# balaji1312/cassnat_asr_public

Measured on AMD Instinct MI355X. Metric: utterances_per_sec, higher is better.
Workload: dtype bf16; 1 GPU; BASELINE configs[1]: CASS-NAT 12L-enc / 1+3+2 dec blocks, d_model 256, 4 heads, d_ff 2048, V 5000, greedy NAST; 32 utterances x 1000 frames x 80 fbank per GPU per step; batch_per_gpu=32, frames=1000, feat_dim=80, global_batch=32, parallelism=utterance-sharded x1, decode_pipelines_per_gpu=2, batches_per_engine_pass=10, utterances_per_engine_pass=320, row_predictions=208, row_predictions_missed=0

## Files before the change

cassnat_asr_public_amd/abi.py:

```python
import ctypes as C
import os
import re

HEADER_PATH = os.path.join(os.path.dirname(os.path.dirname(os.path.abspath(__file__))), "include", "cassnat_hip.h")
SCALARS = {"int": C.c_int, "int32_t": C.c_int32, "int64_t": C.c_int64, "uint64_t": C.c_uint64, "float": C.c_float, "double": C.c_double}
_BASE = re.compile(r"(?:const\s+)?(\w+)\s*")
_DECL = re.compile(r"((?:\*\s*)*)(\w*)\s*(?:\[(\d+)\])?")


class AbiError(ValueError):
    pass


class Abi:
    def __init__(self):
        self.functions, self.structs, self.constants, self.opaque = {}, {}, {}, set()

    def ctype(self, base, stars, where):
        if not stars and base in SCALARS:
            return SCALARS[base]
        if stars == 1 and base == "char":
            return C.c_char_p
        if stars == 1 and base in self.structs:
            return C.POINTER(self.structs[base])
        if stars and (base in SCALARS or base in self.structs or base in self.opaque or base in ("void", "char", "uint8_t")):
            return C.c_void_p
        raise AbiError(f"{where}: unknown type {base + '*' * stars!r}")

    def declarators(self, text, where):
        text = " ".join(text.split())
        m = _BASE.match(text)
        out = []
        for part in text[m.end():].split(",") if m else ():
            d = _DECL.fullmatch(part.strip())
            if not d:
                raise AbiError(f"{where}: cannot read {text!r}")
            if m.group(1) == "void" and not d.group(1) and not d.group(2):
                out.append(("", None))
                continue
            t = self.ctype(m.group(1), d.group(1).count("*"), f"{where}: {text!r}")
            out.append((d.group(2), t * int(d.group(3)) if d.group(3) else t))
        if not out:
            raise AbiError(f"{where}: cannot read {text!r}")
        return out


def parse(text, base=None):
    abi = Abi()
    if base is not None:
        abi.structs.update(base.structs)
        abi.opaque.update(base.opaque)
    text = re.sub(r"/\*.*?\*/|//[^\n]*", " ", text, flags=re.S)
    for name, value in re.findall(r"^[ \t]*#[ \t]*define[ \t]+(CN_\w+)[ \t]+(-?\w+)[ \t]*$", text, re.M):
        abi.constants[name] = int(value, 0)
    text = re.sub(r'^[ \t]*#[^\n]*|extern\s+"C"\s*\{', " ", text, flags=re.M)

    def enum(m):
        for item in filter(None, (s.strip() for s in m.group(1).split(","))):
            name, eq, value = (s.strip() for s in item.partition("="))
            if not eq or not re.fullmatch(r"\w+", name):
                raise AbiError(f"enum: cannot read {item!r}")
            abi.constants[name] = int(value, 0)
        return " "

    def struct(m):
        fields = []
        for line in filter(None, (s.strip() for s in m.group(2).split(";"))):
            got = abi.declarators(line, f"struct {m.group(1)}")
            if any(not name or t is None for name, t in got):
                raise AbiError(f"struct {m.group(1)}: cannot read {line!r}")
            fields += got
        cls = "".join(p.title() for p in m.group(1).split("_"))
        abi.structs[m.group(1)] = type(cls, (C.Structure,), {"_fields_": fields, "__doc__": f"{m.group(1)} of include/cassnat_hip.h"})
        return " "

    text = re.sub(r"\benum\s*\{(.*?)\}\s*;", enum, text, flags=re.S)
    abi.opaque.update(re.findall(r"\btypedef\s+struct\s+(\w+)\s+\1\s*;", text))
    text = re.sub(r"\btypedef\s+struct\s+(\w+)\s+\1\s*;", " ", text)
    text = re.sub(r"\btypedef\s+struct\s+(\w+)\s*\{(.*?)\}\s*\1\s*;", struct, text, flags=re.S)
    for stmt in filter(None, (s.strip() for s in text.split(";"))):
        m = re.fullmatch(r"(.*?)\b(cn_\w+)\s*\((.*)\)", stmt, re.S)
        if not m:
            if stmt == "}":
                continue
            raise AbiError(f"cannot split the declaration {' '.join(stmt.split())!r}")
        name, params = m.group(2), m.group(3).strip()
        ret = abi.declarators(m.group(1), f"{name}: return type")
        args = [] if params == "void" else [d for p in params.split(",") for d in abi.declarators(p, name)]
        if len(ret) != 1 or ret[0][0] or any(not n or t is None for n, t in args):
            raise AbiError(f"cannot split the declaration of {name}: {' '.join(stmt.split())!r}")
        abi.functions[name] = (ret[0][1], [t for _, t in args])
    return abi


with open(HEADER_PATH) as _f:
    HEADER = parse(_f.read())
FUNCTIONS, STRUCTS, CONSTANTS = HEADER.functions, HEADER.structs, HEADER.constants
EXTRA_HEADER_PATH = os.path.join(os.path.dirname(HEADER_PATH), "cassnat_hip_ctc_ngram.h")
with open(EXTRA_HEADER_PATH) as _f:
    EXTRA_FUNCTIONS = parse(_f.read(), base=HEADER).functions


def bind(L):
    for name, (restype, argtypes) in list(FUNCTIONS.items()) + list(EXTRA_FUNCTIONS.items()):
        fn = getattr(L, name)
        fn.restype, fn.argtypes = restype, argtypes
    return L
```

cassnat_asr_public_amd/build.py:

```python
import os
import shutil
import subprocess
import sys
from concurrent.futures import ThreadPoolExecutor

CSRC = os.path.join(os.path.dirname(os.path.abspath(__file__)), "csrc")
LIB = os.path.join(os.path.dirname(os.path.abspath(__file__)), "libcassnat_hip.so")
LIB_F16 = os.path.join(os.path.dirname(os.path.abspath(__file__)), "libcassnat_hip_f16.so")
SOURCES = ["gemm.hip", "fbank.hip", "resample.hip", "flac.hip", "conv2.hip", "conv1.hip", "rowops.hip", "attention.hip", "ctc_align.hip", "ctc_beam.hip", "fused.hip", "fused_x3.hip", "genmax.hip", "proj_x3.hip", "conformer.hip", "chain.hip", "ast.hip", "natlm.hip", "ctc_lm.hip", "ngram.hip", "ctc_ngram.hip", "model.hip", "handle.hip", "weights.hip", "workspace.hip", "sublayers.hip", "decode_ar.hip", "ops.hip"]
FLAGS = ["--offload-arch=gfx950", "-O3", "-std=c++17", "-fPIC", "-Wall", "-Wno-unused-function"]
FILE_FLAGS = {"conv1.hip": ["-mllvm", "-amdgpu-mfma-vgpr-form=1"]}


def _hipcc():
    return shutil.which("hipcc") or "/opt/rocm/bin/hipcc"


def _stale(target, deps):
    if not os.path.exists(target):
        return True
    t = os.path.getmtime(target)
    return any(os.path.getmtime(d) > t for d in deps)


def build(force=False, verbose=False, extra_flags=(), lib=LIB, objdir=None):
    headers = [os.path.join(CSRC, h) for h in os.listdir(CSRC) if h.endswith(".h")]
    headers += [os.path.join(os.path.dirname(CSRC), "..", "include", h) for h in ("cassnat_hip.h", "cassnat_hip_ctc_ngram.h")]
    objdir = objdir or os.path.join(CSRC, "build")
    os.makedirs(objdir, exist_ok=True)

    def compile_one(src):
        obj = os.path.join(objdir, src.replace(".hip", ".o"))
        path = os.path.join(CSRC, src)
        if force or _stale(obj, [path] + headers):
            cmd = [_hipcc()] + FLAGS + FILE_FLAGS.get(src, []) + list(extra_flags) + ["-c", path, "-o", obj]
            if verbose:
                print(" ".join(cmd), file=sys.stderr)
            r = subprocess.run(cmd, capture_output=True, text=True)
            if r.returncode != 0:
                raise RuntimeError(f"hipcc failed on {src}:\n{r.stderr}")
        return obj

    with ThreadPoolExecutor(max_workers=min(6, len(SOURCES))) as ex:
        objs = list(ex.map(compile_one, SOURCES))
    if force or _stale(lib, objs):
        cmd = [_hipcc(), "--offload-arch=gfx950", "-shared", "-fPIC", "-o", lib] + objs
        r = subprocess.run(cmd, capture_output=True, text=True)
        if r.returncode != 0:
            raise RuntimeError(f"link failed:\n{r.stderr}")
    return lib


def build_f16(force=False, verbose=False):
    return build(force=force, verbose=verbose, extra_flags=["-DCN_OP16_F16"], lib=LIB_F16, objdir=os.path.join(CSRC, "build_f16"))


def build_all(force=False, verbose=False):
    return build(force=force, verbose=verbose), build_f16(force=force, verbose=verbose)


def experiments_lib(extra_flags=(), tag="exp"):
    root = os.path.join(os.path.dirname(os.path.dirname(os.path.abspath(__file__))), "ab")
    os.makedirs(root, exist_ok=True)
    return build(extra_flags=["-DCASSNAT_EXPERIMENTS"] + list(extra_flags), lib=os.path.join(root, "libcassnat_hip_%s.so" % tag),
                 objdir=os.path.join(root, "obj_" + tag))


if __name__ == "__main__":
    if "--experiments" in sys.argv:
        print(experiments_lib())
        sys.exit(0)
    for path in build_all(force="--force" in sys.argv, verbose=True):
        print(path)
```

cassnat_asr_public_amd/csrc/attention.hip:

```cpp
#include <cstdlib>

#include <cstdio>
#include <cstdlib>

#include "kernels.h"

struct AttnParams {
    const unsigned char* Q;
    const unsigned char* K;
    const unsigned char* V;
    void* O;
    long long ldq_b, ldk_b, ldv_b;
    int ldo;
    int H, Lq, Lk;
    const unsigned char* keymask;
    int kv_mod;
    int stamps;
    const int* kv_index;
    const int* klen;
    int o_blk;
    int q_blk, kv_blk;
    int q_col, k_col, v_col, q_n, kv_n;
    const int* kcap;
    int kcap_stride;
    const int* iv;
    int iv_stride;
    int causal;
    float scale;
    const float* rel_pos;
    const float* rel_u;
    const float* rel_v;
    int rel_R, ld_pos;
    const int* row_off;
    int kv_packed;
};

template <typename T> struct AttnCfg;
template <> struct AttnCfg<bf16> {
    static constexpr int KROW = 128;
    static constexpr int VROW = 192;
    static constexpr int CPR = 8;
    __device__ static int swz(int row) { return (row >> 1) & 7; }
};
template <> struct AttnCfg<float> {
    static constexpr int KROW = 256;
    static constexpr int VROW = 256;
    static constexpr int CPR = 16;
    __device__ static int swz(int row) { return row & 15; }
};

template <> struct AttnCfg<split_t> {
    static constexpr int KROW = 256;
    static constexpr int VROW = 192;
    static constexpr int CPR = 16;
    __device__ static int swz(int row) { return row & 15; }
};

__device__ long long attn_stamps[8];
#define AT_STAMP(i) if (p.stamps && blockIdx.x == 0 && blockIdx.y == gridDim.y - 1 && blockIdx.z == gridDim.z - 1 && threadIdx.x == 0) attn_stamps[i] = (long long)__builtin_amdgcn_s_memtime();

template <typename T, int NW, bool RES, bool REL = false, bool PK = false>
__global__ __launch_bounds__(64 * NW, (RES && NW == 8) ? 4 : ((__is_same(T, split_t) && NW == 4 && !REL) ? 2 : 1)) void attention_kernel(AttnParams p) {
    typedef AttnCfg<T> Cfg;
    typedef typename Frag<T>::type frag_t;
    constexpr bool SPLIT = __is_same(T, split_t);
    static_assert(!SPLIT || !RES, "split-bf16 attention: the staged forms only");
    constexpr int KROW = Cfg::KROW, CPR = Cfg::CPR;
    constexpr int VROW = RES ? 128 : Cfg::VROW;
    constexpr int KT_BYTES = 64 * KROW, VT_BYTES = (SPLIT ? 2 : 1) * 64 * VROW, NRES = RES ? 4 : 1;
    constexpr int NF = SPLIT ? 4 : KROW / 32;
    constexpr int NT = 64 * NW;
    constexpr int ST_IT = 64 * CPR / NT;

    __shared__ __attribute__((aligned(16))) unsigned char Ks_all[NRES * KT_BYTES];
    __shared__ __attribute__((aligned(16))) unsigned char Vs_all[NRES * VT_BYTES];
    __shared__ __attribute__((aligned(16))) unsigned int Ms_all[NRES * 16];
    __shared__ unsigned int Mplain[NRES];

    const int tid = threadIdx.x, lane = tid & 63, wave = tid >> 6;
    const int half = lane >> 5, l31 = lane & 31;
    const int b = blockIdx.z, h = blockIdx.y;
    AT_STAMP(0)
    const long long q0 = PK ? (long long)p.row_off[b] : (long long)b * p.Lq;
    const int Lq = PK ? p.row_off[b + 1] - p.row_off[b] : p.Lq;
    if constexpr (PK) {
        if ((int)blockIdx.x * (32 * NW) >= Lq) return;
    }
    const int q_row = blockIdx.x * (32 * NW) + wave * 32 + l31;
    const bool wave_active = (blockIdx.x * (32 * NW) + wave * 32) < Lq;
    const int qc = q_row < Lq ? q_row : Lq - 1;

    frag_t qf[NF];
    {
        const unsigned char* qp = p.Q + (q0 + qc) * p.ldq_b + (long long)h * KROW;
        if constexpr (SPLIT) {
#pragma unroll
            for (int s = 0; s < NF; ++s) {
                const unsigned char* c = qp + (s >> 1) * 128 + (2 * (s & 1) + half) * 16;
                qf[s].hi = as_frag<bf16>(ld16(c));
                qf[s].lo = as_frag<bf16>(ld16(c + 64));
            }
        } else if constexpr (PK) {
            const long long qm = q0 + qc;
#pragma unroll
            for (int s = 0; s < NF; ++s) {
                const unsigned char* src = qp + (2 * s + half) * 16;
                src = p.q_blk ? p.Q + cn_blk16_off(qm, p.q_col + h * 64 + (2 * s + half) * 8, p.q_n) : src;
                qf[s] = as_frag<T>(ld16(src));
            }
        } else if (p.q_blk) {
            const long long qm = q0 + qc;
#pragma unroll
            for (int s = 0; s < NF; ++s) qf[s] = as_frag<T>(ld16(p.Q + cn_blk16_off(qm, p.q_col + h * 64 + (2 * s + half) * 8, p.q_n)));
        } else {
#pragma unroll
            for (int s = 0; s < NF; ++s) qf[s] = as_frag<T>(ld16(qp + (2 * s + half) * 16));
        }
    }
    constexpr int REL_N = REL ? 64 : 1;
    __shared__ float rel_tab[REL ? 64 * 64 : 1];
    __shared__ float rel_bias[REL ? NW : 1][32][REL_N];
    if constexpr (REL) {
        constexpr int E = SPLIT ? 8 : Frag<T>::ELEMS;
        const int nr = 2 * p.rel_R + 1;
        for (int i = tid; i < nr * 64; i += NT) rel_tab[i] = p.rel_pos[(long long)(i >> 6) * p.ld_pos + h * 64 + (i & 63)];
        __syncthreads();
        auto dim_of = [&](int s, int j) -> int {
            if constexpr (SPLIT) return 32 * (s >> 1) + 16 * (s & 1) + 8 * half + j;
            else return (2 * s + half) * E + j;
        };
        float qv[NF][E];
#pragma unroll
        for (int s = 0; s < NF; ++s)
#pragma unroll
            for (int j = 0; j < E; ++j) {
                const int dim = dim_of(s, j);
                if constexpr (SPLIT) {
                    const float q = (float)qf[s].hi[j] + (float)qf[s].lo[j];
                    qv[s][j] = q + p.rel_v[h * 64 + dim];
                    const float qu = q + p.rel_u[h * 64 + dim];
                    const bf16 hi = (bf16)qu;
                    qf[s].hi[j] = hi;
                    qf[s].lo[j] = (bf16)(qu - (float)hi);
                } else {
                    const float q = to_f32(qf[s][j]);
                    qv[s][j] = q + p.rel_v[h * 64 + dim];
                    qf[s][j] = from_f32<T>(q + p.rel_u[h * 64 + dim]);
                }
            }
        for (int r = 0; r < nr; ++r) {
            float acc = 0.f;
#pragma unroll
            for (int s = 0; s < NF; ++s)
#pragma unroll
                for (int j = 0; j < E; ++j) acc = fmaf(qv[s][j], rel_tab[r * 64 + dim_of(s, j)], acc);
            acc += __shfl_xor(acc, 32);
            if (half == 0) rel_bias[wave][l31][r] = acc;
        }
        __syncthreads();
    }
    int iv_s1 = 0, iv_e1 = 0, iv_s2 = 0, iv_e2 = 0;
    if (p.iv) {
        const int4 r = *reinterpret_cast<const int4*>(p.iv + ((long long)b * p.iv_stride + qc) * 4);
        iv_s1 = r.x;
        iv_e1 = r.y;
        iv_s2 = r.z;
        iv_e2 = r.w;
    }
    const int klen = p.klen ? p.klen[b] : p.Lk;
    unsigned char* Ks = Ks_all;
    unsigned char* Vs = Vs_all;
    unsigned int* Ms = Ms_all;

    uint4 k_reg[ST_IT], v_reg[ST_IT];
    const int bk = p.kv_index ? p.kv_index[b] : (p.kv_mod > 0 ? b % p.kv_mod : b);
    const bool kpk = PK && p.kv_packed;
    const long long k0 = kpk ? (long long)p.row_off[bk] : (long long)bk * p.Lk;
    const int krows = kpk ? p.row_off[bk + 1] - p.row_off[bk] : p.Lk;
    int kcap = p.kcap ? p.kcap[(long long)bk * p.kcap_stride] : p.Lk;
    if (krows < kcap) kcap = krows;
    const int kvalid = kcap < p.Lk ? kcap : p.Lk;
    const int nkt = kvalid > 0 ? (kvalid + 63) / 64 : 1;
    const unsigned char* kbase = p.K + k0 * p.ldk_b + (long long)h * KROW;
    const unsigned char* vbase = p.V + k0 * p.ldv_b + (long long)h * KROW;
    auto load_tile = [&](int kt) {
#pragma unroll
        for (int i = 0; i < ST_IT; ++i) {
            const int cidx = tid + NT * i;
            const int row = cidx / CPR, ch = cidx % CPR;
            const int key = kt * 64 + row;
            if (key < krows) {
                if (p.kv_blk) {
                    const long long km = k0 + key;
                    k_reg[i] = ld16(p.K + cn_blk16_off(km, p.k_col + h * 64 + ch * 8, p.kv_n));
                    v_reg[i] = ld16(p.V + cn_blk16_off(km, p.v_col + h * 64 + ch * 8, p.kv_n));
                } else {
                    k_reg[i] = ld16(kbase + (long long)key * p.ldk_b + ch * 16);
                    v_reg[i] = ld16(vbase + (long long)key * p.ldv_b + ch * 16);
                }
            } else {
                k_reg[i] = make_uint4(0, 0, 0, 0);
                v_reg[i] = make_uint4(0, 0, 0, 0);
            }
        }
    };
    auto store_tile = [&](int kt) {
#pragma unroll
        for (int i = 0; i < ST_IT; ++i) {
            const int cidx = tid + NT * i;
            const int row = cidx / CPR, ch = cidx % CPR;
            st16(Ks + row * KROW + ((ch ^ Cfg::swz(row)) << 4), k_reg[i]);
            if constexpr (SPLIT)
                st16(Vs + ((ch >> 2) & 1) * 64 * VROW + row * VROW + ((((ch >> 3) << 2) | (ch & 3)) << 4), v_reg[i]);
            else
                st16(Vs + row * VROW + (ch << 4), v_reg[i]);
        }
        if (tid < 64) {
            const int key = kt * 64 + tid;
            unsigned char code = 2;
            if (key < kcap) {
                bool ok = key < klen;
                if (p.keymask) ok = ok && p.keymask[(long long)bk * p.Lk + key] != 0;
                code = ok ? 1 : 0;
            }
            reinterpret_cast<unsigned char*>(Ms)[tid] = code;
            const unsigned long long bad0 = __ballot(code == 0), bad2 = __ballot(code == 2);
            if (tid == 0) Mplain[0] = 1u | (bad2 != 0ull ? 2u : 0u) | (bad0 != 0ull ? 4u : 0u);
        }
    };

    f32x16 o_acc[2];
#pragma unroll
    for (int d = 0; d < 2; ++d)
#pragma unroll
        for (int r = 0; r < 16; ++r) o_acc[d][r] = 0.f;
    float m_run = CN_NEG_FILL, l_run = 0.f;

    if constexpr (RES) {
        const int wave_u = __builtin_amdgcn_readfirstlane(wave);
        const int r8 = lane >> 3, cp = lane & 7;
        for (int piece = wave_u; piece < nkt * 16; piece += NW) {
            const int kt2 = piece >> 4, is_v = (piece >> 3) & 1, j = piece & 7;
            const int row = 8 * j + r8;
            int key = kt2 * 64 + row;
            if (key >= krows) key = krows - 1;
            const int chunk = is_v ? (cp ^ (((row >> 1) & 1) << 2)) : (cp ^ Cfg::swz(row));
            const unsigned char* src;
            if (p.kv_blk)
                src = (is_v ? p.V : p.K) + cn_blk16_off(k0 + key, (is_v ? p.v_col : p.k_col) + h * 64 + chunk * 8, p.kv_n);
            else
                src = is_v ? vbase + (long long)key * p.ldv_b + (chunk << 4) : kbase + (long long)key * p.ldk_b + (chunk << 4);
            unsigned char* dst = (is_v ? Vs_all + kt2 * VT_BYTES : Ks_all + kt2 * KT_BYTES) + j * 1024;
            __builtin_amdgcn_global_load_lds((const __attribute__((address_space(1))) void*)src,
                                             (__attribute__((address_space(3))) void*)dst, 16, 0, 0);
        }
        AT_STAMP(1)
        if (tid < NRES) Mplain[tid] = 1;
        __syncthreads();
        for (int i = tid; i < nkt * 64; i += NT) {
            unsigned char code = 2;
            if (i < kcap) {
                bool ok = i < klen;
                if (p.keymask) ok = ok && p.keymask[(long long)bk * p.Lk + i] != 0;
                code = ok ? 1 : 0;
            }
            reinterpret_cast<unsigned char*>(Ms_all)[i] = code;
            if (code != 1) atomicOr(&Mplain[i >> 6], code == 2 ? 2u : 4u);
        }
        asm volatile("s_waitcnt vmcnt(0)" ::: "memory");
        __syncthreads();
        AT_STAMP(2)
    } else {
        load_tile(0);
    }
    for (int kt = 0; kt < nkt; ++kt) {
        if constexpr (RES) {
            Ks = Ks_all + kt * KT_BYTES;
            Vs = Vs_all + kt * VT_BYTES;
            Ms = Ms_all + kt * 16;
        } else {
            __syncthreads();
            store_tile(kt);
            __syncthreads();
            if (kt + 1 < nkt) load_tile(kt + 1);
        }
        if (!wave_active) continue;

        const unsigned tile_class = Mplain[RES ? kt : 0];
        const bool simple = !REL && !p.iv && !p.causal && (tile_class & 4u) == 0;
#pragma unroll
        for (int sub = 0; sub < 2; ++sub) {
            if (simple && kt * 64 + sub * 32 >= kcap) continue;
            f32x16 sc;
#pragma unroll
            for (int r = 0; r < 16; ++r) sc[r] = 0.f;
            {
                const int row = sub * 32 + l31;
#pragma unroll
                for (int s = 0; s < NF; ++s) {
                    if constexpr (SPLIT) {
                        const int chunk = (s >> 1) * 8 + 2 * (s & 1) + half;
                        split_frag kf;
                        kf.hi = as_frag<bf16>(ld16(Ks + row * KROW + ((chunk ^ Cfg::swz(row)) << 4)));
                        kf.lo = as_frag<bf16>(ld16(Ks + row * KROW + (((chunk + 4) ^ Cfg::swz(row)) << 4)));
                        sc = mfma_frag(kf, qf[s], sc);
                    } else {
                        const int chunk = 2 * s + half;
                        const frag_t kf = as_frag<T>(ld16(Ks + row * KROW + ((chunk ^ Cfg::swz(row)) << 4)));
                        sc = mfma_frag(kf, qf[s], sc);
                    }
                }
            }
            float psum = 0.f, alpha;
            const bool plain = simple && kt * 64 + sub * 32 + 32 <= kcap;
            if (simple) {
                float tmax;
                if (plain) {
                    tmax = sc[0];
#pragma unroll
                    for (int r = 1; r < 16; ++r) tmax = fmaxf(tmax, sc[r]);
                } else {
                    const int k0 = kt * 64 + sub * 32 + 4 * half;
                    tmax = -INFINITY;
#pragma unroll
                    for (int r = 0; r < 16; ++r) {
                        sc[r] = k0 + 8 * (r >> 2) + (r & 3) < kcap ? sc[r] : -INFINITY;
                        tmax = fmaxf(tmax, sc[r]);
                    }
                }
                tmax = xhalf_max(tmax) * p.scale;
                const float m_new = fmaxf(m_run, tmax);
                alpha = __expf(m_run - m_new);
                m_run = m_new;
                const float c2 = p.scale * 1.44269504088896340736f, mb = m_new * 1.44269504088896340736f;
#pragma unroll
                for (int r = 0; r < 16; ++r) {
                    const float pv = __builtin_amdgcn_exp2f(fmaf(sc[r], c2, -mb));
                    sc[r] = pv;
                    psum += pv;
// ... 147 lines not shown
            }
        }
        return;
    }
    if (q_row < Lq) {
        T* orow = reinterpret_cast<T*>(p.O) + (q0 + q_row) * p.ldo + h * 64;
#pragma unroll
        for (int d = 0; d < 2; ++d) {
#pragma unroll
            for (int g = 0; g < 4; ++g) {
                const int dk0 = 32 * d + 8 * g + 4 * half;
                if constexpr (SPLIT) {
                    float o[4];
#pragma unroll
                    for (int e = 0; e < 4; ++e) o[e] = o_acc[d][4 * g + e] * inv;
                    bf16x4 hi, lo;
                    cn_split4(o, hi, lo);
                    unsigned char* ob = reinterpret_cast<unsigned char*>(orow) + cn_split_off((size_t)dk0);
                    *reinterpret_cast<bf16x4*>(ob) = hi;
                    *reinterpret_cast<bf16x4*>(ob + 64) = lo;
                } else if constexpr (sizeof(T) == 2) {
                    bf16x4 o;
#pragma unroll
                    for (int e = 0; e < 4; ++e) o[e] = (bf16)(o_acc[d][4 * g + e] * inv);
                    *reinterpret_cast<bf16x4*>(orow + dk0) = o;
                } else {
                    f32x4 o;
#pragma unroll
                    for (int e = 0; e < 4; ++e) o[e] = o_acc[d][4 * g + e] * inv;
                    *reinterpret_cast<f32x4*>(orow + dk0) = o;
                }
            }
        }
    }
    AT_STAMP(4)
}

int attention_print_stamps() {
    long long h[8];
    CN_HIP_CHECK(hipMemcpyFromSymbol(h, HIP_SYMBOL(attn_stamps), sizeof(h)));
    static const char* names[] = {"", "Q fragments + K/V requests", "K/V landed + mask codes", "key-tile loop", "normalise + store"};
    for (int i = 1; i < 5; ++i) fprintf(stderr, "[attention stamps] %-28s %8lld ticks\n", names[i], h[i] - h[i - 1]);
    fprintf(stderr, "[attention stamps] total %lld ticks (s_memtime)\n", h[4] - h[0]);
    return 0;
}

template <typename T> static int run_attention(const AttnArgs& a, hipStream_t s) {
    constexpr bool PKT = sizeof(T) == 2 && !__is_same(T, split_t);
    AttnParams p;
    p.Q = (const unsigned char*)a.Q;
    p.K = (const unsigned char*)a.K;
    p.V = (const unsigned char*)a.V;
    p.O = a.O;
    p.ldq_b = (long long)a.ldq * sizeof(T);
    p.ldk_b = (long long)a.ldk * sizeof(T);
    p.ldv_b = (long long)a.ldv * sizeof(T);
    p.ldo = a.ldo;
    p.H = a.H;
    p.Lq = a.Lq;
    p.Lk = a.Lk;
    p.keymask = a.keymask;
    p.kv_mod = a.kv_mod;
    static const int stamps = cn_exp_env("CASSNAT_ATTN_STAMPS") ? 1 : 0;
    p.stamps = stamps;
    p.kv_index = a.kv_index;
    p.klen = a.klen;
    p.kcap = a.kcap;
    p.kcap_stride = a.kcap_stride;
    p.o_blk = a.o_blocked;
    p.q_blk = a.q_blocked;
    p.kv_blk = a.kv_blocked;
    p.q_col = a.q_col;
    p.k_col = a.k_col;
    p.v_col = a.v_col;
    p.q_n = a.q_n;
    p.kv_n = a.kv_n;
    if ((a.q_blocked || a.kv_blocked || a.o_blocked) && (sizeof(T) != 2 || __is_same(T, split_t) || a.rel_pos || (a.q_blocked && a.q_n % 32) ||
                                          (a.kv_blocked && a.kv_n % 32) || (a.o_blocked && a.ldo % 32))) {
        cn_set_error("attention: blocked operands exist for the bf16 kernels without relative positions; column counts % 32 == 0");
        return -1;
    }
    p.row_off = a.row_off;
    p.kv_packed = a.kv_packed;
    if ((a.row_off && (a.rel_pos || sizeof(T) != 2 || __is_same(T, split_t))) ||
        (a.kv_packed && (!a.row_off || a.kv_mod > 0 || a.kv_index || a.keymask || a.Lq != a.Lk))) {
        cn_set_error("attention: packed rows exist for the 16-bit kernels without relative positions; packed keys are the entry's own "
                     "rows (self attention without a key mask, kv_mod or kv_index)");
        return -1;
    }
    p.iv = a.intervals;
    p.iv_stride = a.iv_stride;
    p.causal = a.causal;
    p.scale = a.scale;
    p.rel_pos = a.rel_pos;
    p.rel_u = a.rel_u;
    p.rel_v = a.rel_v;
    p.rel_R = a.rel_R;
    p.ld_pos = a.ld_pos;
    {
        if (a.rel_pos) {
            if (a.rel_R < 0 || a.rel_R > 31 || !a.rel_u || !a.rel_v || a.Lq != a.Lk) {
                cn_set_error("attention: relative positions need self attention and max_relative_len <= 31");
                return -1;
            }
            hipLaunchKernelGGL((attention_kernel<T, 2, false, true>), dim3(cn_ceil_div(a.Lq, 64), a.H, a.B), dim3(128), 0, s, p);
            CN_HIP_CHECK(hipGetLastError());
            return 0;
        }
    }
    const long long big_grid = (long long)cn_ceil_div(a.Lq, 128) * a.H * a.B;
    if constexpr (sizeof(T) == 2) {
        static const int no_res = cn_exp_env("CASSNAT_ATTN_NO_RES") ? 1 : 0;
        if (a.Lk <= 256 && !no_res) {
            static const int nw = cn_exp_env("CASSNAT_ATTN_NW") ? atoi(cn_exp_env("CASSNAT_ATTN_NW")) : 0;
            const int use = nw ? nw : (a.Lq > 128 ? 8 : (a.Lq > 64 ? 4 : 2));
            if (a.row_off) {
                if (use >= 8)
                    hipLaunchKernelGGL((attention_kernel<T, 8, true, false, PKT>), dim3(cn_ceil_div(a.Lq, 256), a.H, a.B), dim3(512), 0, s, p);
                else if (use >= 4)
                    hipLaunchKernelGGL((attention_kernel<T, 4, true, false, PKT>), dim3(cn_ceil_div(a.Lq, 128), a.H, a.B), dim3(256), 0, s, p);
                else
                    hipLaunchKernelGGL((attention_kernel<T, 2, true, false, PKT>), dim3(cn_ceil_div(a.Lq, 64), a.H, a.B), dim3(128), 0, s, p);
            } else if (use >= 8)
                hipLaunchKernelGGL((attention_kernel<T, 8, true>), dim3(cn_ceil_div(a.Lq, 256), a.H, a.B), dim3(512), 0, s, p);
            else if (use >= 4)
                hipLaunchKernelGGL((attention_kernel<T, 4, true>), dim3(cn_ceil_div(a.Lq, 128), a.H, a.B), dim3(256), 0, s, p);
            else
                hipLaunchKernelGGL((attention_kernel<T, 2, true>), dim3(cn_ceil_div(a.Lq, 64), a.H, a.B), dim3(128), 0, s, p);
            CN_HIP_CHECK(hipGetLastError());
            return 0;
        }
    }
    if (a.row_off) {
        if (big_grid >= 1024)
            hipLaunchKernelGGL((attention_kernel<T, 4, false, false, PKT>), dim3(cn_ceil_div(a.Lq, 128), a.H, a.B), dim3(256), 0, s, p);
        else
            hipLaunchKernelGGL((attention_kernel<T, 2, false, false, PKT>), dim3(cn_ceil_div(a.Lq, 64), a.H, a.B), dim3(128), 0, s, p);
    } else if (big_grid >= 1024)
        hipLaunchKernelGGL((attention_kernel<T, 4, false>), dim3(cn_ceil_div(a.Lq, 128), a.H, a.B), dim3(256), 0, s, p);
    else
        hipLaunchKernelGGL((attention_kernel<T, 2, false>), dim3(cn_ceil_div(a.Lq, 64), a.H, a.B), dim3(128), 0, s, p);
    CN_HIP_CHECK(hipGetLastError());
    return 0;
}

int launch_attention(int prec, const AttnArgs& a, hipStream_t s) {
    if (a.B <= 0 || a.Lq <= 0 || a.Lk <= 0 || a.H <= 0) return 0;
    const size_t es = cn_elem_size(prec);
    if ((a.ldq * es) % 16 || (a.ldk * es) % 16 || (a.ldv * es) % 16 || (a.ldo * es) % 16) {
        cn_set_error("attention: row strides must keep rows 16-byte aligned");
        return -1;
    }
    if (prec == CN_PREC_X3) {
        if (a.ldq % 32 || a.ldk % 32 || a.ldv % 32 || a.ldo % 32) {
            cn_set_error("attention: split-bf16 rows need strides that are multiples of 32 elements");
            return -1;
        }
    }
    const long long w = 64LL * a.H;
    if ((!a.q_blocked && a.ldq < w) || (!a.kv_blocked && (a.ldk < w || a.ldv < w)) || a.ldo < w) {
        cn_set_error("attention: row strides ldq / ldk / ldv / ldo must be >= 64 * H");
        return -1;
    }
    if (a.rel_pos && a.ld_pos < w) {
        cn_set_error("attention: the relative-position table needs ld_pos >= 64 * H");
        return -1;
    }
    auto bad_window = [w](int col, int n) { return col < 0 || col % 8 || col + w > n; };
    if ((a.q_blocked && bad_window(a.q_col, a.q_n)) ||
        (a.kv_blocked && (bad_window(a.k_col, a.kv_n) || bad_window(a.v_col, a.kv_n)))) {
        cn_set_error("attention: a blocked operand's columns col .. col + 64 * H - 1 must lie inside its q_n / kv_n columns "
                     "(col >= 0, col % 8 == 0)");
        return -1;
    }
    if (prec == CN_PREC_X3) return run_attention<split_t>(a, s);
    return prec == CN_PREC_F32 ? run_attention<float>(a, s) : run_attention<bf16>(a, s);
}
```

cassnat_asr_public_amd/csrc/chain.hip:

```cpp
#include <cstdio>
#include <cstdlib>
#include <algorithm>
#include <cmath>
#include <cstring>
#include <vector>

#include "kernels.h"

constexpr int CH_D = 256;
constexpr int CH_UNIT_BYTES = 16384;
constexpr int CH_RING = 8;
constexpr int CH_TAB_FLOATS = 5120;
constexpr int CH_TAB_BYTES = CH_TAB_FLOATS * 4;
constexpr int CH_LDS = CH_TAB_BYTES + CH_RING * CH_UNIT_BYTES;
static_assert(CH_LDS <= 160 * 1024, "LDS budget");
constexpr int CT_BO = 0, CT_LN1A = 256, CT_LN1B = 512, CT_B2 = 768, CT_NLNA = 1024, CT_NLNB = 1280, CT_BT = 1536,
              CT_B1 = 3072;
constexpr int CH_MAX_TAIL = 48, CH_MAX_FFN_TILES = 64;

__device__ long long ch_stamps[16];

typedef unsigned u32x4 __attribute__((ext_vector_type(4)));
typedef int v4i __attribute__((ext_vector_type(4)));
typedef int v8i __attribute__((ext_vector_type(8)));

struct ChainParams {
    float* x;
    const bf16* ctx;
    int ldctx;
    const uint4* wstream;
    const float* tab;
    bf16* out;
    int ldo;
    bf16* ln_out;
    int ld_ln;
    int M, ffn_tiles, tail_tiles, has_next;
    float eps;
    int stamps;
    int stamp_block;
    int x_in_blk, x_out_blk, store_x;
    int out_blk;
    int ctx_blk;
    const int* f8_q;
    const int* m_dev;
};

#define CH_STR2(x) #x
#define CH_STR(x) CH_STR2(x)
#define CH_DMA(src, dst)                                                                              \
    __builtin_amdgcn_global_load_lds((const __attribute__((address_space(1))) void*)(src),          \
                                     (__attribute__((address_space(3))) void*)(dst), 16, 0, 0)
#define CH_READ8(F, addr, OFFK)                                                                       \
    asm volatile("ds_read_b128 %0, %8 offset:" CH_STR(((OFFK) + 0) * 1024) "\n\t"                     \
                 "ds_read_b128 %1, %8 offset:" CH_STR(((OFFK) + 1) * 1024) "\n\t"                     \
                 "ds_read_b128 %2, %8 offset:" CH_STR(((OFFK) + 2) * 1024) "\n\t"                     \
                 "ds_read_b128 %3, %8 offset:" CH_STR(((OFFK) + 3) * 1024) "\n\t"                     \
                 "ds_read_b128 %4, %8 offset:" CH_STR(((OFFK) + 4) * 1024) "\n\t"                     \
                 "ds_read_b128 %5, %8 offset:" CH_STR(((OFFK) + 5) * 1024) "\n\t"                     \
                 "ds_read_b128 %6, %8 offset:" CH_STR(((OFFK) + 6) * 1024) "\n\t"                     \
                 "ds_read_b128 %7, %8 offset:" CH_STR(((OFFK) + 7) * 1024)                            \
                 : "=&v"(F[0]), "=&v"(F[1]), "=&v"(F[2]), "=&v"(F[3]), "=&v"(F[4]), "=&v"(F[5]),      \
                   "=&v"(F[6]), "=&v"(F[7])                                                           \
                 : "v"(addr)                                                                          \
                 : "memory")
#define CH_WAIT8(F)                                                                                   \
    asm volatile("s_waitcnt lgkmcnt(0)"                                                               \
                 : "+v"(F[0]), "+v"(F[1]), "+v"(F[2]), "+v"(F[3]), "+v"(F[4]), "+v"(F[5]), "+v"(F[6]), "+v"(F[7]) \
                 :: "memory")
__device__ __forceinline__ void ch_tab4_nowait(unsigned addr, f32x4& a, f32x4& b, f32x4& c, f32x4& d) {
    asm volatile("ds_read_b128 %0, %4\n\t"
                 "ds_read_b128 %1, %4 offset:32\n\t"
                 "ds_read_b128 %2, %4 offset:64\n\t"
                 "ds_read_b128 %3, %4 offset:96"
                 : "=&v"(a), "=&v"(b), "=&v"(c), "=&v"(d)
                 : "v"(addr)
                 : "memory");
}
template <typename D>
__device__ __forceinline__ void ch_tab4_nowait_after(unsigned addr, const D& dep, f32x4& a, f32x4& b, f32x4& c, f32x4& d) {
    asm volatile("ds_read_b128 %0, %4\n\t"
                 "ds_read_b128 %1, %4 offset:32\n\t"
                 "ds_read_b128 %2, %4 offset:64\n\t"
                 "ds_read_b128 %3, %4 offset:96"
                 : "=&v"(a), "=&v"(b), "=&v"(c), "=&v"(d)
                 : "v"(addr), "v"(dep)
                 : "memory");
}
template <typename D>
__device__ __forceinline__ void ch_tab4(unsigned addr, const D& dep, f32x4& a, f32x4& b, f32x4& c, f32x4& d) {
    asm volatile("ds_read_b128 %0, %4\n\t"
                 "ds_read_b128 %1, %4 offset:32\n\t"
                 "ds_read_b128 %2, %4 offset:64\n\t"
                 "ds_read_b128 %3, %4 offset:96\n\t"
                 "s_waitcnt lgkmcnt(0)"
                 : "=&v"(a), "=&v"(b), "=&v"(c), "=&v"(d)
                 : "v"(addr), "v"(dep)
                 : "memory");
}

#define CH_SB0_ __builtin_amdgcn_sched_barrier(0)
#define CH_LGKM_WAIT4(N, a, b, c, d) asm volatile("s_waitcnt lgkmcnt(" #N ")" : "+v"(a), "+v"(b), "+v"(c), "+v"(d) :: "memory")

template <bool ADD>
__device__ __forceinline__ void ch_layernorm_pack(f32x16 (&acc)[8], unsigned tab_lane, int off_a, int off_b, int off_add,
                                                  float eps, bf16x8 (&bop)[16]) {
    float s = 0.f;
#pragma unroll
    for (int nt = 0; nt < 8; ++nt)
#pragma unroll
        for (int r = 0; r < 16; ++r) s += acc[nt][r];
    s += __shfl_xor(s, 32);
    const float mean = s / (float)CH_D;
    float ss = 0.f;
#pragma unroll
    for (int nt = 0; nt < 8; ++nt)
#pragma unroll
        for (int r = 0; r < 16; ++r) ss = fmaf(acc[nt][r] - mean, acc[nt][r] - mean, ss);
    ss += __shfl_xor(ss, 32);
    const float inv = 1.0f / (sqrtf(ss / (float)(CH_D - 1)) + eps);
    f32x4 ga[2][4], be[2][4], ad[2][4];
    CH_SB0_;
    ch_tab4_nowait_after(tab_lane + off_a * 4, inv, ga[0][0], ga[0][1], ga[0][2], ga[0][3]);
    ch_tab4_nowait(tab_lane + off_b * 4, be[0][0], be[0][1], be[0][2], be[0][3]);
    if constexpr (ADD) ch_tab4_nowait(tab_lane + off_add * 4, ad[0][0], ad[0][1], ad[0][2], ad[0][3]);
#pragma unroll
    for (int nt = 0; nt < 8; ++nt) {
        const int c = nt & 1, n = c ^ 1;
// ... 621 lines not shown
        CH_ACT_GAP(HAS_OLD, XO, 5)                                                                             \
        CH_M1(XN, Fa[6], bop[6]);                                                                              \
        CH_ACT_GAP(HAS_OLD, XO, 6)                                                                             \
        CH_M1(XN, Fa[7], bop[7]);                                                                              \
        CH_ACT_GAP(HAS_OLD, XO, 7)                                                                             \
        CH_BLK1("+", "v", "%[c]", XN, Fb, bop, 8, Fa, RA_B, RK_B, CH_PRE_B_##k(M0OFF), CH_DMA0(SOFF), CH_DMA1, CH_DMA2, \
                CH_DMA3, SB, CH_NODRAIN);                                                                      \
        ch_tab4_nowait(tabb(TNEXT), b1v[0], b1v[1], b1v[2], b1v[3]);
#define CH_W2N(k, RA_A, RK_A, RA_B, RK_B, M0OFF, SOFF, SB, PREA, POST)                                        \
        CH_BLK2(acc, Fa, pb[0], Fb, RA_A, RK_A, PREA, "", "", "", "", SB, CH_NODRAIN);                         \
        CH_BLK2(acc, Fb, pb[1], Fa, RA_B, RK_B, CH_PRE_B_##k(M0OFF), CH_DMA0(SOFF), CH_DMA1, CH_DMA2, CH_DMA3, SB, POST);
#define CH_FFN_GROUP(FIRST, LAST)                                                                              \
        {                                                                                                      \
            const uint4* sb_cur = group_base(gpos);                                                            \
            const uint4* sb_next = group_base(gpos + 1);                                                       \
            const int t0 = 4 * g;                                                                              \
            if constexpr (FIRST) {                                                                             \
                CH_W1N(0, ra0, 8, ra0, 16, 0x1C000, 0x1C000, sb_cur, xh0, xh1, false, 1)                       \
                 \
                 \
                 \
                asm volatile("s_nop 13\n\ts_nop 13\n\ts_waitcnt lgkmcnt(0)" : "+v"(xh0), "+v"(b1v[0]), "+v"(b1v[1]), "+v"(b1v[2]), "+v"(b1v[3]), "+v"(Fa[0]), \
                             "+v"(Fa[1]), "+v"(Fa[2]), "+v"(Fa[3]), "+v"(Fa[4]), "+v"(Fa[5]), "+v"(Fa[6]), "+v"(Fa[7]) :: "memory"); \
            } else {                                                                                           \
                CH_W2N(0, ra0, 8, ra0, 16, 0x1C000, 0x1C000, sb_cur, CH_PRE_A4, CH_NODRAIN)                    \
            }                                                                                                  \
            CH_W1N(1, ra0, 24, ra0, 32, 0x0, 0x0, sb_next, xh1, xh0, true, t0 + 2)                             \
            CH_W2N(2, ra0, 40, ra0, 48, 0x4000, 0x4000, sb_next, CH_PRE_A4, CH_NODRAIN)                        \
            CH_W1N(3, ra0, 56, ra1, 0, 0x8000, 0x8000, sb_next, xh0, xh1, true, t0 + 3)                        \
            CH_W2N(4, ra1, 8, ra1, 16, 0xC000, 0xC000, sb_next, CH_PRE_A4, CH_NODRAIN)                         \
            CH_W1N(5, ra1, 24, ra1, 32, 0x10000, 0x10000, sb_next, xh1, xh0, true, t0 + 4)                     \
            CH_W2N(6, ra1, 40, ra1, 48, 0x14000, 0x14000, sb_next, CH_PRE_A4, CH_NODRAIN)                      \
            if constexpr (!(LAST)) {                                                                           \
                CH_W1N(7, ra1, 56, ra0, 0, 0x18000, 0x18000, sb_next, xh0, xh1, true, t0 + 5)                  \
            } else {                                                                                           \
                 \
                 \
                 \
                asm volatile("" : "+v"(xh1));                                                                  \
                CH_SB0;                                                                                        \
                _Pragma("unroll") for (int i = 0; i < 8; ++i) CH_ACT_PIECE(xh1, i)                             \
                CH_SB0;                                                                                        \
                CH_W2N(7, ra1, 56, ra0, 0, 0x18000, 0x18000, sb_next, CH_PRE_A, CH_DRAIN "s_waitcnt lgkmcnt(0)\n\t") \
            }                                                                                                  \
            ++g;                                                                                               \
            ++gpos;                                                                                            \
        }
        int g = 0;
        if (G_FFN == 1) {
            CH_FFN_GROUP(true, true)
        } else {
            CH_FFN_GROUP(true, false)
            while (g < G_FFN - 1) CH_FFN_GROUP(false, false)
            CH_FFN_GROUP(false, true)
        }
#undef CH_FFN_GROUP
#undef CH_W1N
#undef CH_W2N
#undef CH_ACT_GAP
#undef CH_ACT_PIECE
        CH_LAND_FRAGMENTS("");
        asm volatile("s_waitcnt lgkmcnt(0)" : "+v"(b1v[0]), "+v"(b1v[1]), "+v"(b1v[2]), "+v"(b1v[3]) :: "memory");
    }
    CH_STAMP(5)

    if (p.store_x && (p.x_out_blk ? rb < nrb : live)) {
        float* xp = p.x_out_blk ? p.x + (long long)rb * 8192 + 4 * lane : p.x + (long long)m * CH_D + 4 * half;
        const int step = p.x_out_blk ? 256 : 8;
#pragma unroll
        for (int nt = 0; nt < 8; ++nt)
#pragma unroll
            for (int g = 0; g < 4; ++g) {
                f32x4 o;
#pragma unroll
                for (int e = 0; e < 4; ++e) o[e] = acc[nt][4 * g + e];
                *reinterpret_cast<f32x4*>(xp + step * (4 * nt + g)) = o;
            }
    }
    CH_STAMP(6)
    if (p.has_next) {
        ch_layernorm_pack<false>(acc, tab_lane, CT_NLNA, CT_NLNB, 0, p.eps, bop);
        CH_STAMP(7)
        if (p.ln_out) {
            if (live) {
                bf16* op = p.ln_out + (long long)m * p.ld_ln + 4 * half;
#pragma unroll
                for (int k = 0; k < 16; ++k)
#pragma unroll
                    for (int q = 0; q < 2; ++q) {
                        bf16x4 o;
#pragma unroll
                        for (int e = 0; e < 4; ++e) o[e] = bop[k][4 * q + e];
                        *reinterpret_cast<bf16x4*>(op + 16 * k + 8 * q) = o;
                    }
            }
        }
        if (G_TAIL > 0) {
            f32x16 q0, q1;
            f32x4 btv[4];
            bf16x4 o_[4];
            u32x4 w_[2];
            const int NTT = 8 * G_TAIL;
            auto tabt = [&](int tt) -> unsigned { return tab_lane + (unsigned)((CT_BT + 32 * (tt < NTT ? tt : NTT - 1)) * 4); };
            bf16* op16 = p.out + (long long)m * p.ldo + 8 * half;
            unsigned char* ob16 = reinterpret_cast<unsigned char*>(p.out) + (long long)rb * (p.ldo >> 5) * 2048 + lane * 16;
            unsigned char* st_base = p.out_blk ? ob16 : reinterpret_cast<unsigned char*>(op16);
            const int st_tile = p.out_blk ? 2048 : 64, st_half = p.out_blk ? 1024 : 32;
            const bool st_on = (p.out_blk ? rb < nrb : live) && p.stamps != 2;
            ch_tab4_nowait(tabt(0), btv[0], btv[1], btv[2], btv[3]);
            CH_READ8(Fa, ra0, 0);
            asm volatile("s_waitcnt lgkmcnt(0)" : "+v"(btv[0]), "+v"(btv[1]), "+v"(btv[2]), "+v"(btv[3]), "+v"(Fa[0]), "+v"(Fa[1]),
                         "+v"(Fa[2]), "+v"(Fa[3]), "+v"(Fa[4]), "+v"(Fa[5]), "+v"(Fa[6]), "+v"(Fa[7]) :: "memory");
#define CH_TAIL_STORE(v, ptr) *(ptr) = (v)
#define CH_EPI_CVT(QO, g0)                                                                                     \
            {                                                                                                  \
                _Pragma("unroll") for (int g_ = (g0); g_ < (g0) + 2; ++g_)                                     \
                    _Pragma("unroll") for (int e = 0; e < 4; ++e) o_[g_][e] = (bf16)QO[4 * g_ + e];             \
                asm volatile("" : "+v"(o_[g0]), "+v"(o_[(g0) + 1]));                                            \
            }
#define CH_EPI_OUT(TT, gp)                                                                                     \
            {                                                                                                  \
                const uint2 lo_ = __builtin_bit_cast(uint2, o_[2 * (gp)]), hi_ = __builtin_bit_cast(uint2, o_[2 * (gp) + 1]); \
                const auto s0_ = __builtin_amdgcn_permlane32_swap(lo_.x, hi_.x, false, false);                 \
                const auto s1_ = __builtin_amdgcn_permlane32_swap(lo_.y, hi_.y, false, false);                 \
                w_[gp] = u32x4{s0_[0], s1_[0], s0_[1], s1_[1]};                                                \
                if (st_on) CH_TAIL_STORE(w_[gp], reinterpret_cast<u32x4*>(st_base + (long long)(TT) * st_tile + (gp) * st_half)); \
                else asm volatile("" :: "v"(w_[gp]));                                                          \
            }
#define CH_EPI_GAP(HAS_OLD, CODE)                                                                              \
            CH_SB0;                                                                                            \
            if constexpr (HAS_OLD) CODE                                                                        \
            CH_SB0;
#define CH_S5N(k, RA_A, RK_A, RA_B, RK_B, M0OFF, SOFF, SB, QN, QO, HAS_OLD)                                    \
            QN = __builtin_shufflevector(__builtin_shufflevector(btv[0], btv[1], 0, 1, 2, 3, 4, 5, 6, 7),      \
                                         __builtin_shufflevector(btv[2], btv[3], 0, 1, 2, 3, 4, 5, 6, 7),      \
                                         0, 1, 2, 3, 4, 5, 6, 7, 8, 9, 10, 11, 12, 13, 14, 15);   \
            CH_M1R(CH_PRE_A, QN, Fa[0], bop[0], Fb[0], Fb[1], RA_A, (RK_A) + 0);                               \
            CH_SB0;                                                                                            \
            ch_tab4_nowait(tabt(8 * g + (k) + 1), btv[0], btv[1], btv[2], btv[3]);   \
            CH_SB0;                                                                                            \
            CH_M1R("", QN, Fa[1], bop[1], Fb[2], Fb[3], RA_A, (RK_A) + 2);                                     \
            CH_SB0;                                                                                            \
            CH_M1R("", QN, Fa[2], bop[2], Fb[4], Fb[5], RA_A, (RK_A) + 4);                                     \
            CH_EPI_GAP(HAS_OLD, CH_EPI_CVT(QO, 0))                                                             \
            CH_M1R("", QN, Fa[3], bop[3], Fb[6], Fb[7], RA_A, (RK_A) + 6);                                     \
            CH_EPI_GAP(HAS_OLD, CH_EPI_CVT(QO, 2))                                                             \
            CH_M1(QN, Fa[4], bop[4]);                                                                          \
            CH_EPI_GAP(HAS_OLD, CH_EPI_OUT(8 * g + (k) - 1, 0))                                                \
            CH_M1(QN, Fa[5], bop[5]);                                                                          \
            CH_EPI_GAP(HAS_OLD, CH_EPI_OUT(8 * g + (k) - 1, 1))                                                \
            CH_M1(QN, Fa[6], bop[6]);                                                                          \
            CH_SB0;                                                                                            \
            CH_M1(QN, Fa[7], bop[7]);                                                                          \
            CH_SB0;                                                                                            \
            CH_BLK1("+", "v", "%[c]", QN, Fb, bop, 8, Fa, RA_B, RK_B, CH_PRE_B_##k(M0OFF), CH_DMA0(SOFF), CH_DMA1, CH_DMA2, \
                    CH_DMA3, SB, CH_NODRAIN);
#define CH_TAIL_GROUP(FIRST, LAST)                                                                             \
            {                                                                                                  \
                const uint4* sb_cur = group_base(gpos);                                                        \
                const uint4* sb_next = group_base(gpos + 1);                                                   \
                CH_S5N(0, ra0, 8, ra0, 16, 0x1C000, 0x1C000, sb_cur, q0, q1, !(FIRST))                         \
                CH_S5N(1, ra0, 24, ra0, 32, 0x0, 0x0, sb_next, q1, q0, true)                                   \
                CH_S5N(2, ra0, 40, ra0, 48, 0x4000, 0x4000, sb_next, q0, q1, true)                             \
                CH_S5N(3, ra0, 56, ra1, 0, 0x8000, 0x8000, sb_next, q1, q0, true)                              \
                CH_S5N(4, ra1, 8, ra1, 16, 0xC000, 0xC000, sb_next, q0, q1, true)                              \
                CH_S5N(5, ra1, 24, ra1, 32, 0x10000, 0x10000, sb_next, q1, q0, true)                           \
// ... 2 lines not shown
                if constexpr (LAST) {                                                                          \
                       \
                    CH_LAND_FRAGMENTS("");                                                                     \
                    asm volatile(CH_DRAIN : "+v"(q1));                                                         \
                    CH_SB0;                                                                                    \
                    CH_EPI_CVT(q1, 0) CH_EPI_CVT(q1, 2) CH_EPI_OUT(8 * g + 7, 0) CH_EPI_OUT(8 * g + 7, 1)      \
                    CH_SB0;                                                                                    \
                }                                                                                              \
                ++g;                                                                                           \
                ++gpos;                                                                                        \
            }
            int g = 0;
            if (G_TAIL == 1) {
                CH_TAIL_GROUP(true, true)
            } else {
                CH_TAIL_GROUP(true, false)
                while (g < G_TAIL - 1) CH_TAIL_GROUP(false, false)
                CH_TAIL_GROUP(false, true)
            }
#undef CH_TAIL_GROUP
#undef CH_S5N
#undef CH_EPI_GAP
#undef CH_EPI_OUT
#undef CH_EPI_CVT
            CH_LAND_FRAGMENTS("");
            asm volatile("s_waitcnt lgkmcnt(0)" : "+v"(btv[0]), "+v"(btv[1]), "+v"(btv[2]), "+v"(btv[3]) :: "memory");
        }
    }
    CH_STAMP(8)
    asm volatile("s_waitcnt vmcnt(0) lgkmcnt(0)" ::: "memory");
    CH_STAMP(9)
    if (p.stamps && (int)blockIdx.x == p.stamp_block && tid == 0) ch_stamps[11] = (long long)__builtin_amdgcn_s_memrealtime();
}

int chain_print_stamps() {
    long long h[16];
    CN_HIP_CHECK(hipMemcpyFromSymbol(h, HIP_SYMBOL(ch_stamps), sizeof(h)));
    static const char* names[] = {"prologue issue", "x/ctx landed + acc", "first unit visible", "S1 out-proj", "LN1 + b2",
                                  "S3 ffn loop", "S4 x store", "LNn", "S5 tail", "drain"};
    for (int i = 1; i < 10; ++i) fprintf(stderr, "[chain stamps] %-20s %8lld ticks\n", names[i], h[i] - h[i - 1]);
    fprintf(stderr, "[chain stamps] total %lld ticks (s_memtime)\n", h[9] - h[0]);
    fprintf(stderr, "[chain stamps] wall %.2f us (s_memrealtime) -> %.0f MHz\n", (h[11] - h[10]) / 100.0,
            (double)(h[9] - h[0]) / ((h[11] - h[10]) / 100.0));
    return 0;
}

int launch_chain(const ChainArgs& a, hipStream_t s) {
    if (a.f8 && (a.swish || a.dff <= 0 || a.dff % 256 != 0 || !a.f8_q)) {
        cn_set_error("chain: the e4m3 feed-forward form needs d_ff % 256 == 0 and the ReLU activation");
        return -1;
    }
    if (a.d != CH_D || a.dff < 0 || a.dff % 128 != 0 || a.dff / 32 > CH_MAX_FFN_TILES || a.tail_n < 0 || a.tail_n % 256 != 0 ||
        a.tail_n / 32 > CH_MAX_TAIL || (a.tail_n > 0 && (!a.has_next || !a.out)) || (a.has_next && !a.out && !a.ln_out)) {
        cn_set_error("chain: needs d_model == 256, d_ff % 128 == 0 <= 2048, tail width % 256 == 0 <= 1536");
        return -1;
    }
    if (a.M <= 0) return 0;
    ChainParams p;
    p.x = a.x;
    p.ctx = reinterpret_cast<const bf16*>(a.ctx);
    p.ldctx = a.ldctx;
    p.wstream = reinterpret_cast<const uint4*>(a.wstream);
    p.tab = a.tab;
    p.out = reinterpret_cast<bf16*>(a.out);
    p.ldo = a.ldo;
    p.ln_out = reinterpret_cast<bf16*>(a.ln_out ? a.ln_out : (a.tail_n == 0 ? a.out : nullptr));
    p.ld_ln = a.ln_out ? a.ld_ln : a.ldo;
    p.M = a.M;
    p.m_dev = a.m_dev;
    p.ffn_tiles = a.dff / 32;
    p.tail_tiles = a.tail_n / 32;
    p.has_next = a.has_next;
    p.eps = a.eps;
    static const int stamps = cn_exp_env("CASSNAT_CHAIN_STAMPS") ? atoi(cn_exp_env("CASSNAT_CHAIN_STAMPS")) : 0;
    p.stamps = stamps;
    static const int stamp_block = cn_exp_env("CASSNAT_CHAIN_STAMP_BLOCK") ? atoi(cn_exp_env("CASSNAT_CHAIN_STAMP_BLOCK")) : 0;
    p.stamp_block = stamp_block;
    p.x_in_blk = a.x_in_blocked;
    p.x_out_blk = a.x_out_blocked;
    p.store_x = a.store_x && (a.ctx || a.dff);
    p.out_blk = a.out_blocked && a.tail_n > 0;
    p.ctx_blk = a.ctx && a.ctx_blocked;
    p.f8_q = a.f8_q;
    if (p.ctx_blk && a.ldctx != CH_D) {
        cn_set_error("chain: a blocked ctx has 256 columns");
        return -1;
    }
    if (p.out_blk && a.ldo % 32 != 0) {
        cn_set_error("chain: a blocked tail output needs ldo % 32 == 0");
        return -1;
    }
    static CnAttrOnce attr_once;
    int attr_dev;
    if (attr_once.need(&attr_dev)) {
        CN_HIP_CHECK(hipFuncSetAttribute((const void*)chain_kernel<false, false>, hipFuncAttributeMaxDynamicSharedMemorySize, CH_LDS));
        CN_HIP_CHECK(hipFuncSetAttribute((const void*)chain_kernel<true, false>, hipFuncAttributeMaxDynamicSharedMemorySize, CH_LDS));
        CN_HIP_CHECK(hipFuncSetAttribute((const void*)chain_kernel<false, true>, hipFuncAttributeMaxDynamicSharedMemorySize, CH_LDS));
        CN_HIP_CHECK(hipFuncSetAttribute((const void*)chain_kernel<false, false, true>, hipFuncAttributeMaxDynamicSharedMemorySize, CH_LDS));
        CN_HIP_CHECK(hipFuncSetAttribute((const void*)chain_kernel<false, true, true>, hipFuncAttributeMaxDynamicSharedMemorySize, CH_LDS));
        attr_once.mark(attr_dev);
    }
    if (a.m_dev) {
        if (a.swish) {
            cn_set_error("chain: a device-side row count exists for the ReLU forms (the transformer decoder side)");
            return -1;
        }
        if (a.f8)
            hipLaunchKernelGGL((chain_kernel<false, true, true>), dim3(cn_ceil_div(p.M, 128)), dim3(256), CH_LDS, s, p);
        else
            hipLaunchKernelGGL((chain_kernel<false, false, true>), dim3(cn_ceil_div(p.M, 128)), dim3(256), CH_LDS, s, p);
    } else if (a.f8)
        hipLaunchKernelGGL((chain_kernel<false, true>), dim3(cn_ceil_div(p.M, 128)), dim3(256), CH_LDS, s, p);
    else if (a.swish)
        hipLaunchKernelGGL((chain_kernel<true, false>), dim3(cn_ceil_div(p.M, 128)), dim3(256), CH_LDS, s, p);
    else
        hipLaunchKernelGGL((chain_kernel<false, false>), dim3(cn_ceil_div(p.M, 128)), dim3(256), CH_LDS, s, p);
    CN_HIP_CHECK(hipGetLastError());
    return 0;
}

static inline uint16_t ch_bf16_bits(float f) { return cn_host_op16(f); }

size_t chain_stream_units(int has_outproj, int dff, int tail_n, int f8) {
    return (has_outproj ? 8 : 0) + (f8 ? 1 : 2) * (dff / 32) + tail_n / 32;
}

static void ch_pack_rows(const float* w, int ld, int rt, bool acc_order, uint16_t* out) {
    for (int f = 0; f < 16; ++f)
        for (int lane = 0; lane < 64; ++lane)
            for (int j = 0; j < 8; ++j) {
                const int k = acc_order ? 32 * (f >> 1) + 16 * (f & 1) + 8 * (j >> 2) + 4 * (lane >> 5) + (j & 3)
                                        : 16 * f + 8 * (lane >> 5) + j;
                out[((size_t)f * 64 + lane) * 8 + j] = ch_bf16_bits(w[(size_t)(32 * rt + (lane & 31)) * ld + k]);
            }
}
static void ch_pack_w2(const float* w2, int dff, int t, uint16_t* out) {
    for (int s = 0; s < 2; ++s)
        for (int nt = 0; nt < 8; ++nt)
            for (int lane = 0; lane < 64; ++lane)
                for (int j = 0; j < 8; ++j)
                    out[((size_t)(8 * s + nt) * 64 + lane) * 8 + j] = ch_bf16_bits(
                        w2[(size_t)(32 * nt + (lane & 31)) * dff + 32 * t + 16 * s + 8 * (j >> 2) + 4 * (lane >> 5) + (j & 3)]);
}
unsigned char cn_f32_to_e4m3_host(float f) {
    const unsigned char sign = std::signbit(f) ? 0x80 : 0;
    float a = std::fabs(f);
    if (a != a) return 0x7f;
    if (a >= 448.f) return sign | 0x7e;
    if (a < 0.0009765625f) return sign;
    int e;
    (void)std::frexp(a, &e);
    int E = e - 1;
    if (E < -6) {
        const int r = (int)std::nearbyint(a * 512.f);
        return sign | (unsigned char)(r >= 8 ? 0x08 : r);
    }
    int r = (int)std::nearbyint((a / std::ldexp(1.f, E) - 1.f) * 8.f);
    if (r == 8) {
        r = 0;
        ++E;
    }
    const int bits = ((E + 7) << 3) | r;
    return sign | (unsigned char)(bits > 0x7e ? 0x7e : bits);
}
int cn_e4m3_exp(float mx) { return mx > 0.f ? (int)std::floor(std::log2(448.f / mx)) : 0; }

// ... 73 lines not shown
```

cassnat_asr_public_amd/csrc/kernels.h:

```cpp
#pragma once
#include "common.h"

enum { CN_PREC_F32 = 0, CN_PREC_BF16 = 1, CN_PREC_X3 = 3 };
static inline size_t cn_elem_size(int prec) { return prec == CN_PREC_BF16 ? 2 : 4; }

enum { CN_EPI_RELU = 1, CN_EPI_RESID = 2, CN_EPI_EMBED = 4, CN_EPI_SWISH = 8 };
struct GemmArgs {
    const void* A = nullptr;
    int lda = 0;
    const void* W = nullptr;
    const float* bias = nullptr;
    void* C = nullptr;
    int ldc = 0;
    int c_f32 = 0;
    int M = 0, N = 0, K = 0;
    int epi = 0;
    const float* resid = nullptr;
    float resid_scale = 1.0f;
    int ldr = 0;
    const float* pe = nullptr;
    int pe_period = 1;
    float scale = 1.f;
    int ab_fp8 = 0;
    float acc_scale = 1.f;
// ... 6 lines not shown
};
int launch_gemm(int prec, const GemmArgs& a, hipStream_t s);

struct UttMeta {
    int frames;
    int tp;
    int sub_lo;
    int sub_hi;
};
int launch_conv1(int prec, const float* x, const float* w9c, const float* bias, void* out, int B, int T, int F, int T1,
                 int F1, int C, int halo, hipStream_t s, const UttMeta* utt_meta = nullptr);
int launch_conv1_planes(const float* x, const float* w9c, const float* bias, void* out, int B, int T, int F, int T1, int F1,
                        int C, int halo, hipStream_t s, const UttMeta* utt_meta = nullptr);
int launch_conv1_mixplanes(const float* x, const float* w9c, const float* bias, void* out, int B, int T, int F, int T1, int F1, int C,
                           int halo, float scale_l, float scale_q, hipStream_t s, const UttMeta* utt_meta = nullptr);
int launch_conv1_f8(const float* x, const float* w9c, const float* bias, void* out8, int B, int T, int F, int T1, int F1, int C,
                    int halo, float scale, hipStream_t s, const UttMeta* utt_meta = nullptr);
bool conv1_bordered_bf16_applies(int C, int F1);
int launch_conv1_bordered_bf16(const float* x, const float* w9c, const float* bias, void* out, int B, int T, int F, int T1, int F1,
                               int C, hipStream_t s, const UttMeta* utt_meta = nullptr);
constexpr int CN_MAX_SUB = 64;
struct SubList {
    int n;
    int rows[CN_MAX_SUB];
    int frames[CN_MAX_SUB];
};
int launch_expand_meta(const SubList& subs, UttMeta* meta, int B, hipStream_t s);

int launch_layernorm(int prec, const float* x, const float* a2, const float* b2, void* y, int y_f32, int M, int d,
                     float eps, hipStream_t s);
int launch_layernorm_fp8(const float* x, const float* a2, const float* b2, void* y, int M, int d, float eps, float scale,
                         hipStream_t s);
int launch_quantize_fp8(const void* src_bf16, int ld, void* dst, int M, int K, float scale, hipStream_t s);
int launch_cmvn(float* x, const int* len, const double* mean, const double* sd, int B, int T, int F, hipStream_t s);
int launch_feature_range(const float* x, size_t n, const float* limit, unsigned int* fault, hipStream_t s);
int launch_unpack_rows(const float* packed, const int* off, const int* len, float* out, int rows, int T, int F, float pad,
                       const double* mean, const double* sd, hipStream_t s);
int launch_unpack_compressed(const unsigned char* staged, const int* off, const int* len, const int* kind, float* out, int rows, int T,
                             int F, float pad, const double* mean, const double* sd, hipStream_t s);
int launch_splice_rows(const float* src, const int* off, const int* len, float* out, int rows, int T_out, int F0, int left, int right,
                       int skip, float pad, const double* mean, const double* sd, hipStream_t s);
int launch_logsoftmax_argmax(float* logits, int M, int V, int ldl, int* arg, float* maxlp, int write_logp,
                             hipStream_t s);
int launch_keymask(const float* feats, int B, int T, int F, int Tp, int stride, float padding, unsigned char* km,
                   hipStream_t s);
int launch_fill_queries(const float* table, float* out, int B, int U, int d, hipStream_t s);
int launch_fill_queries_packed(const float* table, float* out, const int* row_off, int B, int cap_rows, int d, hipStream_t s);
int launch_shift_right(const float* x, float* y, int B, int U, int d, hipStream_t s);
int launch_esa_paths(const int* top2_idx, const float* top2_val, const unsigned char* select, float threshold, int* best, int M,
                     int n, hipStream_t s);
int launch_lm_embed(const int* tok, int ld, const float* lut, const float* pe, float* x, int B, int U, int d, float scale,
                    hipStream_t s);
int launch_gather_logp(const float* logp, int V, const int* tgt, int ld, float* out, int B, int U, hipStream_t s);
int launch_fill_int(int* p, size_t n, int v, hipStream_t s);
int launch_copy_rows(void* dst, int dst_ld, const void* src, int src_ld, int width, int rows, hipStream_t s);
int launch_convert(int prec, const float* src, void* dst, size_t n, hipStream_t s);
int launch_convert_back(int prec, const void* src, float* dst, size_t n, hipStream_t s);

struct AttnArgs {
    const void* Q = nullptr;
    const void* K = nullptr;
    const void* V = nullptr;
    void* O = nullptr;
    int ldq = 0, ldk = 0, ldv = 0, ldo = 0;
    int B = 0, H = 0, Lq = 0, Lk = 0;
    const unsigned char* keymask = nullptr;
    int kv_mod = 0;
    const int* kv_index = nullptr;
    const int* klen = nullptr;
    const int* kcap = nullptr;
    int kcap_stride = 1;
    int q_blocked = 0, kv_blocked = 0;
    int q_col = 0, k_col = 0, v_col = 0, q_n = 0, kv_n = 0;
    int o_blocked = 0;
    const int* row_off = nullptr;
    int kv_packed = 0;
    const int* intervals = nullptr;
    int iv_stride = 0;
    int causal = 0;
    float scale = 0.125f;
    const float* rel_pos = nullptr;
    const float *rel_u = nullptr, *rel_v = nullptr;
    int rel_R = 0, ld_pos = 0;
};
int launch_attention(int prec, const AttnArgs& a, hipStream_t s);
int attention_print_stamps();

int launch_glu(int prec, const void* in, void* out, int M, int d, hipStream_t s);
int launch_dwconv(int prec, const void* x, const float* w, const float* bias, float* y, int B, int L, int d, int k, int form,
                  hipStream_t s);
int launch_groupnorm_swish(int prec, const float* x, double* stats, const float* gw, const float* gb, void* out, int B, int L,
                           int d, float eps, hipStream_t s);

struct AlignArgs {
    const int* best = nullptr;
    const unsigned char* keymask = nullptr;
    const float* size_ratio = nullptr;
    int B = 0, Tp = 0, blank = 0, left = 0, right = 0;
    int src_mod = 0;
    int* shift = nullptr;
    int* src_size = nullptr;
    int* ylen = nullptr;
    int* ymax = nullptr;
    int* intervals = nullptr;
    int raw_path = 0;
    const int* ylen_in = nullptr;
    const UttMeta* utt_meta = nullptr;
    int no_trigger = 0;
};
int launch_ctc_align(const AlignArgs& a, hipStream_t s);
int launch_row_plan(const int* ylen, int B, int U, int hyp_stride, int sub, const UttMeta* utt_meta, const int* ymax_dev, int* row_off,
                    hipStream_t s);
int launch_ctc_collapse(const int* best, const unsigned char* km, int B, int Tp, int sos, int pad, int ld, int* tgt, int* len, int* keylen,
                        int* maxlen, hipStream_t s);

struct CtcBeamArgs {
    const float* logp = nullptr;
    const int* top_idx = nullptr;
    const float* size_ratio = nullptr;
    int B = 0, Tp = 0, V = 0, P = 0, W = 0, blank = 0, Lmax = 0;
    double lp = 0.0;
    unsigned char* hist_parent = nullptr;
    int* hist_tok = nullptr;
    int* hyp = nullptr;
    int* hyp_len = nullptr;
    double* score = nullptr;
    double* p_blk = nullptr;
    double* p_nblk = nullptr;
    int* n_out = nullptr;
};
int launch_ctc_prefix_beam(const CtcBeamArgs& a, hipStream_t s);
struct ViterbiArgs {
    const float* logp = nullptr;
    const unsigned char* keymask = nullptr;
    const float* size_ratio = nullptr;
    const int* labels = nullptr;
    const int* label_len = nullptr;
    int B = 0, Tp = 0, V = 0, ld = 0, ymax = 0, blank = 0;
    unsigned char* bp = nullptr;
    int* out_path = nullptr;
};
int launch_ctc_viterbi(const ViterbiArgs& a, hipStream_t s);
int launch_greedy_pack(const int* tok, const float* val, const int* ylen, int B, int U, int sos, int hyp_stride,
                       int* hyp, int* hyp_len, double* score, hipStream_t s, int sub = 0, const UttMeta* utt_meta = nullptr,
                       const int* ymax_dev = nullptr, const int* row_off = nullptr);
int launch_topk(const float* logp, int M, int V, int ldl, int k, int* idx, float* val, hipStream_t s);
int launch_logsoftmax_topk(const float* logits, int M, int V, int ldl, float temperature, int k, int* idx, float* val,
                           hipStream_t s);
int launch_logsoftmax_fuse_topk(const float* att, const float* lm, int M, int V, int ldl, float temperature, float w, int k,
                                int* idx, float* val, hipStream_t s);
int launch_logsoftmax_gather(const float* logits, int M, int V, int ldl, const int* cand, int k, float* out, hipStream_t s);

enum { FF_ACT_RELU = 0, FF_ACT_SWISH = 1 };
struct FfnFusedArgs {
    float* x = nullptr;
    const float *ln_a = nullptr, *ln_b = nullptr;
    const void* w1p = nullptr;
    const float* b1 = nullptr;
    const void* w2p = nullptr;
    const float* b2 = nullptr;
    const float *nln_a = nullptr, *nln_b = nullptr;
    void* xn_out = nullptr;
    int M = 0, d = 0, dff = 0;
    float eps = 1e-6f;
    int nslice = 1;
    float* partial = nullptr;
    int act = FF_ACT_RELU;
};
int launch_ffn_fused(const FfnFusedArgs& a, hipStream_t s);
int launch_ffn_reduce(float* x, const float* partial, int nslice, const float* b2, const float* nln_a, const float* nln_b,
                      void* xn_out, int M, float eps, hipStream_t s);
void pack_ffn_w1(const float* w1, int dff, uint16_t* out);
void pack_ffn_w2(const float* w2, int dff, uint16_t* out);

struct FfnX3Args {
    float* x = nullptr;
    const float *ln_a = nullptr, *ln_b = nullptr;
    const void* wst = nullptr;
    bool mix = false;
    const float *b1 = nullptr, *b2 = nullptr;
    const float *nln_a = nullptr, *nln_b = nullptr;
    void* xn_out = nullptr;
    int M = 0, d = 0, dff = 0;
    float eps = 1e-6f;
    const void* ctx = nullptr;
    int ldctx = 256;
    const void* wo_p = nullptr;
    const float* bo = nullptr;
    const void* tail_p = nullptr;
    const float* tail_b = nullptr;
    void* tail_out = nullptr;
    int tail_n = 0, ld_tail = 0;
    int act = FF_ACT_RELU;
};
bool ffn_x3_applies(int d, int dff);
int launch_ffn_x3(const FfnX3Args& a, hipStream_t s);
size_t ffn_x3_stream_bytes(int dff);
void pack_ffn_x3(const float* w1, const float* w2, int dff, uint16_t* out, bool mix = false);
bool ffn_mix_applies();

struct FbankOpts {
    float sample_rate = 16000.f, frame_length_ms = 25.f, frame_shift_ms = 10.f, preemph = 0.97f, low_freq = 20.f, high_freq = 0.f;
    int num_mel = 80, window_type = 0 , remove_dc = 1, use_power = 1, use_log = 1;
};
int fbank_num_frames(const FbankOpts& o, int num_samples);
int launch_fbank(const FbankOpts& o, const float* wave, const int* num_samples, int B, int max_samples, const float* cmvn_mean,
                 const float* cmvn_istd, float* out, int Tmax, float pad_value, hipStream_t s);
int fbank_frame_samples(const FbankOpts& o);
int launch_fbank_packed(const FbankOpts& o, const unsigned char* staged, long long staged_bytes, const int* off, const int* samples,
                        float* out, int rows, int T, float pad_value, const double* mean, const double* sd, bool f32, hipStream_t s);

long long resample_num_samples(int in_rate, int out_rate, long long in_samples);
int resample_table(int in_rate, int out_rate, int* in_unit, int* out_unit, int* max_taps, int* first, int* taps, float* weights,
                   long long capacity);
int launch_wave_resample(int in_rate, int out_rate, const unsigned char* staged, long long staged_bytes, const int* off, const int* samples,
                         const int* channels, const int* channel, int utts, const int* rows, int n_rows, long long max_out, float* out,
                         const int* out_off, hipStream_t s);

long long flac_scratch_bytes(int frames, long long frame_words);
int launch_flac_decode(const unsigned char* staged, long long staged_bytes, const int* table, int frames, const int* utt, int utts,
                       int max_channels, long long frame_words, unsigned char* pcm, long long pcm_bytes, int* status, int* scratch,
                       hipStream_t s);

bool conv2_dma_applies(int prec, int C, int N);
bool conv2_f8_applies(int C, int N);
int launch_conv2_f8(const void* in8, const void* w8, const int* q8_dev, const float* bias, void* out, int B, int T1, int F1, int T2,
                    int F2, hipStream_t s, float out8_scale = 0.f);
bool linear256_f8_applies(int N, int K);
int launch_linear256_f8(const void* A8, const void* W8, const int* q8_dev, const float* bias, float* out, int M, int K, float scale,
                        const float* pe, int pe_period, hipStream_t s);
bool conv2_mix_applies(int prec, int C, int N);
int launch_conv2_mix(const void* img, const void* w_hi, const void* w8q, const void* w8l, const int* q8_dev, const float* bias, void* out,
                     int B, int T1, int F1, int T2, int F2, hipStream_t s);
constexpr int MIX_LG_AQ = 0, MIX_LG_AL = 11;
int pack_conv2_f8(const float* w, int C, long long s_co, long long s_tap, long long s_ci, unsigned char* out);
void pack_conv2_mix(const float* w, int C, long long s_co, long long s_tap, long long s_ci, unsigned char* out, int* q8);
bool conv2_x3_applies(int prec, int C, int N);
int launch_conv2_x3(const void* in_hi, const void* in_lo, const void* w_hi, const void* w_lo, const float* bias, void* out, int B,
                    int T1, int F1, int T2, int F2, hipStream_t s);
bool linear256_dma_applies(int prec, int N, int K);
int launch_linear256_dma(const void* A, int lda, const void* W, const float* bias, float* out, int M, int K, float scale,
                         const float* pe, int pe_period, hipStream_t s);
int launch_conv2_dma(const void* in, const void* w, const float* bias, void* out, int B, int T1, int F1, int T2, int F2,
                     hipStream_t s);

constexpr int CHAIN_TAB_FLOATS = 5120;
constexpr int CHAIN_UNIT_BYTES = 16384;
struct ChainArgs {
    float* x = nullptr;
    const void* ctx = nullptr;
    int ldctx = 0;
    int ctx_blocked = 0;
    const void* wstream = nullptr;
    const float* tab = nullptr;
    void* out = nullptr;
    int ldo = 0;
    void* ln_out = nullptr;
    int ld_ln = 0;
    int M = 0, d = 0, dff = 0, tail_n = 0, has_next = 0;
    const int* m_dev = nullptr;
    int x_in_blocked = 0, x_out_blocked = 0, store_x = 1;
    int out_blocked = 0;
    int swish = 0;
    int f8 = 0;
    const int* f8_q = nullptr;
    float eps = 1e-6f;
};
int launch_chain(const ChainArgs& a, hipStream_t s);
int chain_print_stamps();
struct ChainWeights {
    const float *wo = nullptr, *bo = nullptr, *ln1_a = nullptr, *ln1_b = nullptr, *w1 = nullptr, *b1 = nullptr, *w2 = nullptr,
                *b2 = nullptr, *nln_a = nullptr, *nln_b = nullptr, *wt = nullptr, *bt = nullptr;
    int dff = 0, tail_n = 0;
};
constexpr float CHAIN_F8_S_LN = 16.f, CHAIN_F8_S_HID = 8.f;
size_t chain_stream_units(int has_outproj, int dff, int tail_n, int f8 = 0);
void pack_chain(const ChainWeights& w, uint16_t* stream, float* tab, int* f8_q = nullptr);
unsigned char cn_f32_to_e4m3_host(float f);
int cn_e4m3_exp(float mx);

struct ProjX3Args {
    const void* A = nullptr;
    int lda = 256;
    const void* wp = nullptr;
    const float* bias = nullptr;
    void* C = nullptr;
    int ldc = 0;
    int c_f32 = 0;
    const float* resid = nullptr;
    int ldr = 0;
    float resid_scale = 1.f;
    int M = 0, N = 0;
};
bool proj_x3_applies(int N, int K);
int launch_proj_x3(const ProjX3Args& a, hipStream_t s);
size_t proj_x3_off(int n, int k);
void pack_proj_x3(const float* w, int N, unsigned char* out);

struct GenmaxArgs {
    const void* h = nullptr;
    const void* wp = nullptr;
    const float* bp = nullptr;
    bool x3 = false;
    int* arg = nullptr;
    float* maxlp = nullptr;
    int M = 0, V = 0, d = 0;
    const int* m_dev = nullptr;
    const int* tgt = nullptr;
    float* tgt_lp = nullptr;
    int tgt_U = 0, tgt_ld = 0;
};
int launch_genmax(const GenmaxArgs& a, hipStream_t s);
int genmax_vtw(int V);
void pack_genmax(const float* w, const float* b, int V, uint16_t* wout, float* bout);
int genmax_x3_vtw(int V);
void pack_genmax_x3(const float* w, const float* b, int V, uint16_t* wout, float* bout);
bool genmax_applies(int prec, int d, int V);

int launch_ast_embed(const int* tok, const float* lut, const float* pe_row, float* x, int n, int d, float scale, hipStream_t s);
int launch_ast_kv_append(int prec, const void* qkv, void* ck, void* cv, int n, int d, int slots, int pos, hipStream_t s);
struct GatherAttnArgs {
    const void* q = nullptr;
    int ldq = 0;
    const void* k = nullptr;
    const void* v = nullptr;
    void* o = nullptr;
    int ldo = 0;
    int n = 0, H = 0, nkeys = 0, slots = 0, d = 0, table_stride = 0;
    const int* anc = nullptr;
    const unsigned char* keyok = nullptr;
    const int* utt = nullptr;
    const unsigned char* keymask = nullptr;
    float scale = 0.125f;
    int append_pos = -1;
};
int launch_ast_gather_attn(int prec, int mode, const GatherAttnArgs& a, hipStream_t s);
int launch_ast_embed_rows(const int* tok, const float* lut, const float* pe, const int* pos, float* x, int n, int d, float scale,
                          int max_pos, hipStream_t s);
struct GatherRowsArgs {
    const void* q = nullptr;
    int ldq = 0;
    void* k = nullptr;
    void* v = nullptr;
    void* o = nullptr;
    int ldo = 0;
// ... 119 lines not shown
```

cassnat_asr_public_amd/csrc/model.h:

```cpp
#pragma once
#include <map>
#include <memory>
#include <string>
#include <vector>

#include "../../include/cassnat_hip.h"
#include "kernels.h"

namespace cn_host {

struct HostTensor {
    std::vector<float> data;
    std::vector<int64_t> shape;
};

struct Linear {
    void* W = nullptr;
    float* b = nullptr;
    int N = 0, K = 0;
    void* W8 = nullptr;
    float* w8_inv = nullptr;
    void* px3 = nullptr;
    void* gm_w = nullptr;
    float* gm_b = nullptr;
// ... 133 lines not shown
    bool kv_blocked = false;
    bool ctx_blocked = false;
    long long call_id = 0;
    int c1_halo_B = -1, c1_halo_T1 = -1;
    bool ctc_maxlp_valid = false;

    void* cv_a = nullptr;
    float* cv_f = nullptr;
    double* gn_stats = nullptr;
    int* ymax_pinned = nullptr;
    const float* op16_feat_limit = nullptr;
    float op16_feat_limit_host = -1.f;
    unsigned int* op16_fault = nullptr;
    std::map<std::string, std::pair<void*, size_t>> scratch;

    float* tgt_lut = nullptr;
    int ast_max_len = 0, ast_slots = 0, ast_ctc_beam = 0, ast_Tp_cap = 0, ast_blank = 0;
    std::vector<void*> ast_kvx, ast_ck, ast_cv;
    float *ast_logits = nullptr, *ast_r0 = nullptr, *ast_r[2] = {nullptr, nullptr}, *ast_maxlp = nullptr;
    int* ast_arg = nullptr;
    std::vector<void*> ast_allocs;
    AstBeamState beam;
    int beam_S = 0, beam_L = 0, beam_K = 0;
    int *beam_idx = nullptr;
    float *beam_val = nullptr, *beam_ctc = nullptr, *beam_lm = nullptr;
    cn_model* ast_lm = nullptr;
    const void* lib_tag = nullptr;

    int B = 0, T = 0, T1 = 0, Tp = 0, U = 0, last_k = 0;
    int att_rows_U = 0;
    int dec_group = 1;
    std::map<std::string, cn_host::Capture> captures;

    bool prof_on = false;
    std::string prof_filter;
    std::vector<hipEvent_t> ev_pool;
    size_t ev_used = 0;
    std::vector<cn_host::ProfPending> prof_pending;
    std::map<std::string, cn_host::ProfStat> prof_stats;
};

namespace cn_host {

struct ProfScope {
    cn_model* m;
    hipStream_t s;
    ProfPending pp;
    bool live = false;
    ProfScope(cn_model* m_, const char* tag, double flops, double bytes, hipStream_t s_) : m(m_), s(s_) {
        if (!m->prof_on) return;
        if (!m->prof_filter.empty() && m->prof_filter.find(std::string("|") + tag + "|") == std::string::npos) return;
        while (m->ev_pool.size() < m->ev_used + 2) {
            hipEvent_t e;
            if (hipEventCreate(&e) != hipSuccess) return;
            m->ev_pool.push_back(e);
        }
        pp.tag = tag;
        pp.a = m->ev_pool[m->ev_used++];
        pp.b = m->ev_pool[m->ev_used++];
        pp.flops = flops;
        pp.bytes = bytes;
        live = hipEventRecord(pp.a, s) == hipSuccess;
    }
    ~ProfScope() {
        if (live && hipEventRecord(pp.b, s) == hipSuccess) m->prof_pending.push_back(pp);
    }
};

int build_weights(cn_model* m);

int build_workspace(cn_model* m);
int ws_check(cn_model* m, int B, int T, int G, const char* what);
int capture(cn_model* m, const char* name, const void* src, bool model_prec, int dtype, std::vector<int64_t> shape, hipStream_t s);
int scratch_buf(cn_model* m, const char* name, size_t bytes, void** out);

int run_linear(cn_model* m, const char* tag, const Linear& l, const void* A, int lda, void* C, int ldc, int c_f32, int M, int epi,
               const float* resid, int ldr, hipStream_t s);
int run_ln(cn_model* m, const Norm& n, const float* x, void* y, int M, hipStream_t s);
int run_ffn(cn_model* m, const Layer& L, const Norm& n, float* x, int M, const Norm* next, void* next_out, hipStream_t s);
bool x3_chain_applies(const cn_model* m, const Layer& L, const Linear* tail);
int run_x3_chain(cn_model* m, const Layer& L, const Norm& n1, float* x, int M, const Norm& next, void* next_out, const Linear* tail,
                 void* tail_out, int ld_tail, const char* tag, hipStream_t s);
int run_self_attn_core(cn_model* m, int B, int Lseq, const unsigned char* keymask, const int* klen, int causal, hipStream_t s,
                       bool blocked = false, const int* row_off = nullptr);
int run_self_attn(cn_model* m, const Layer& L, const Norm* pre, float* x, int B, int Lseq, const unsigned char* keymask,
                  const int* klen, int causal, hipStream_t s);
enum { CHX_IN_BLK = 1, CHX_OUT_BLK = 2, CHX_NO_STORE = 4 };
int run_chain(cn_model* m, const ChainRef& r, float* x, int M, void* out, int ldo, bool with_next, int x_mode, hipStream_t s,
              void* ln_out = nullptr, int ld_ln = 0, bool out_blocked = false, const char* tag = "row_chain",
              const int* m_dev = nullptr);
int run_enc_layer_fp8(cn_model* m, const Layer& L, float* x, int B, int Tp, hipStream_t s);
int run_ffn_swish(cn_model* m, const Linear& w1, const Linear& w2, const Norm& n, float* x, int M, float scale, hipStream_t s);
int run_rel_self_attn(cn_model* m, const Layer& L, const Norm& n, float* x, int B, int Lseq, const unsigned char* keymask,
                      const int* klen, hipStream_t s);
int run_conv_module(cn_model* m, const Layer& L, const Norm& n, float* x, int B, int Lseq, hipStream_t s);
int run_conformer_self_layer(cn_model* m, const Layer& L, float* x, int B, int Lseq, const unsigned char* keymask, const int* klen,
                             hipStream_t s);
int run_conformer_layer_chain(cn_model* m, const Layer& L, float* x, int B, int Lseq, const unsigned char* keymask, const int* klen,
                              bool mixed, int Tp, const int* src_intervals, bool rowmajor, int x_in, int x_out, void* final_out,
                              hipStream_t s);
int run_src_attn_core(cn_model* m, const Layer& L, int B, int U, int Tp, const int* intervals, hipStream_t s, bool q_blocked = false,
                      const int* row_off = nullptr);
int run_src_attn(cn_model* m, const Layer& L, const Norm* pre, float* x, int B, int U, int Tp, const int* intervals, hipStream_t s);
int run_generator(cn_model* m, const Linear& g, const void* h, int M, int* arg, float* maxlp, bool need_rows, hipStream_t s,
                  const int* m_dev = nullptr);

int check_call(cn_model* m, int B, int T, int F, bool area = false);
int stage_encode(cn_model* m, const float* feats, int B, int T, int F, const cn_decode_opts* o, hipStream_t s);
int stage_encode_ctc_rows(cn_model* m, const float* feats, int B, int T, int F, const cn_decode_opts* o, hipStream_t s);

int lm_prepare_buffers(cn_model* lm, int max_len, int max_slots);
int lm_check_step(const cn_model* lm, int max_len, int max_slots, const char* who);
int lm_step_run(cn_model* lm, int n, int pos, const int32_t* tok_dev, const int32_t* anc_dev, const uint8_t* keyok_dev,
                int table_stride, hipStream_t s, const int32_t* row_pos = nullptr, const int32_t* row_stay = nullptr);

}
```

cassnat_asr_public_amd/csrc/model.hip:

```cpp
#include <algorithm>
#include <cmath>

#include "ctc_ngram_search.h"
#include "model.h"

using namespace cn_host;

namespace cn_host {

int check_call(cn_model* m, int B, int T, int F, bool area) {
    if (!m || !m->finalized) {
        cn_set_error("model not finalized");
        return -1;
    }
    if (F != m->cfg.input_size || B < 1 || T < 1 || (!area && (B > m->maxB || T > m->maxT))) {
        cn_set_error("decode: batch/frames/feature dims outside the configured workspace (B=" + std::to_string(B) +
                     " T=" + std::to_string(T) + " F=" + std::to_string(F) + ")");
        return -1;
    }
    return ws_check(m, B, T, 1, "decode");
}

static int stage_encode_align(cn_model* m, const float* feats, const float* ratio, int B, int T, int F,
                              const cn_decode_opts* o, hipStream_t s) {
// ... 86 lines not shown
        g.conv = 1;
        g.cB = B;
        g.cT1 = T1;
        g.cF1 = F1;
        g.cC = d;
        g.cT2 = Tp;
        g.cF2 = F2;
        ProfScope ps(m, "conv2", 2.0 * g.M * g.N * g.K,
                     ((double)B * T1 * F1 * d + (double)g.N * g.K + (double)g.M * g.N) * m->es, s);
        if (mix_planes) {
            const size_t wn = (size_t)d * 9 * d;
            const unsigned char* w = (const unsigned char*)m->conv2_mixw;
            CN_TRY(launch_conv2_mix(m->c1, w, w + 2 * wn, w + 3 * wn, m->conv2_mixq, m->conv2.b, m->c2, B, T1, F1, Tp, F2, s));
        } else if (x3_planes) {
            const size_t img = (size_t)B * (T1 + 2) * (F1 + 2) * d * 2, wpl = (size_t)d * 9 * d * 2;
            CN_TRY(launch_conv2_x3(m->c1, (const unsigned char*)m->c1 + img, m->conv2_x3w, (const unsigned char*)m->conv2_x3w + wpl,
                                   m->conv2.b, m->c2, B, T1, F1, Tp, F2, s));
        } else if (f8_img) {
            CN_TRY(launch_conv2_f8(m->c1, m->conv2_f8w, m->conv2_f8q, m->conv2.b, m->c2, B, T1, F1, Tp, F2, s, f8_lin ? FP8_S_IMG : 0.f));
        } else {
            CN_TRY(launch_gemm(m->prec, g, s));
        }
    }
    if (cap && !f8_lin) CN_TRY(capture(m, "conv2", m->c2, true, CN_DTYPE_F32, {B, Tp, F2, d}, s));
    if (f8_lin) {
        ProfScope ps(m, "linear_out_embed", 2.0 * M * d * (double)F2 * d, (double)M * F2 * d + (double)d * F2 * d + (double)M * d * 4, s);
        CN_TRY(launch_linear256_f8(m->c2, m->linear_f8w, m->linear_f8q, m->linear_out.b, m->x, M, F2 * d, sqrtf((float)d),
                                   c.conf_enc ? nullptr : m->pe, Tp, s));
    } else {
        GemmArgs g;
        g.A = m->c2;
        g.lda = F2 * d;
        g.W = m->linear_out.W;
        g.bias = m->linear_out.b;
        g.C = m->x;
        g.ldc = d;
        g.c_f32 = 1;
        g.M = M;
        g.N = d;
        g.K = F2 * d;
        g.epi = CN_EPI_EMBED;
        g.pe = c.conf_enc ? nullptr : m->pe;
        g.pe_period = Tp;
        g.scale = sqrtf((float)d);
        ProfScope ps(m, "linear_out_embed", 2.0 * g.M * g.N * g.K,
                     ((double)g.M * g.K + (double)g.N * g.K) * m->es + (double)g.M * g.N * 4, s);
        CN_TRY(launch_gemm(m->prec, g, s));
    }
    if (cap) CN_TRY(capture(m, "x_embed", m->x, false, CN_DTYPE_F32, {B, Tp, d}, s));
    static const bool no_chain_c = cn_exp_env("CASSNAT_NO_CHAIN") != nullptr;
    if (c.conf_enc && !m->enc.empty() && m->enc[0].cf_a.w && !no_chain_c) {
        for (size_t n = 0; n < m->enc.size(); ++n) {
            const bool last = n + 1 == m->enc.size();
            const int xin = (cap || n == 0) ? 0 : CHX_IN_BLK, xout = cap ? 0 : (last ? CHX_NO_STORE : CHX_OUT_BLK);
            CN_TRY(run_conformer_layer_chain(m, m->enc[n], m->x, B, Tp, m->keymask, nullptr, false, 0, nullptr, cap, xin, xout,
                                             last ? m->enc_h : nullptr, s));
            if (cap) CN_TRY(capture(m, ("enc_layer" + std::to_string(n)).c_str(), m->x, false, CN_DTYPE_F32, {B, Tp, d}, s));
        }
        if (cap) CN_TRY(capture(m, "enc_h", m->enc_h, true, CN_DTYPE_F32, {B, Tp, d}, s));
        return 0;
    }
    if (c.conf_enc) {
        for (size_t n = 0; n < m->enc.size(); ++n) {
            CN_TRY(run_conformer_self_layer(m, m->enc[n], m->x, B, Tp, m->keymask, nullptr, s));
            if (cap) CN_TRY(capture(m, ("enc_layer" + std::to_string(n)).c_str(), m->x, false, CN_DTYPE_F32, {B, Tp, d}, s));
        }
        CN_TRY(run_ln(m, m->enc_norm, m->x, m->enc_h, M, s));
        if (cap) CN_TRY(capture(m, "enc_h", m->enc_h, true, CN_DTYPE_F32, {B, Tp, d}, s));
        return 0;
    }
    static const bool no_chain = cn_exp_env("CASSNAT_NO_CHAIN") != nullptr;
    if (m->fp8_enc && (m->enc_chain.size() != m->enc.size() || no_chain)) {
        for (size_t n = 0; n < m->enc.size(); ++n) {
            CN_TRY(run_enc_layer_fp8(m, m->enc[n], m->x, B, Tp, s));
            if (cap) CN_TRY(capture(m, ("enc_layer" + std::to_string(n)).c_str(), m->x, false, CN_DTYPE_F32, {B, Tp, d}, s));
        }
        CN_TRY(run_ln(m, m->enc_norm, m->x, m->enc_h, M, s));
        if (cap) CN_TRY(capture(m, "enc_h", m->enc_h, true, CN_DTYPE_F32, {B, Tp, d}, s));
        return 0;
    }
    const bool chain = !m->enc.empty() && m->enc_chain.size() == m->enc.size() && !no_chain;
    static const bool blk = cn_exp_env("CASSNAT_NO_BLOCKED_QKV") == nullptr;
    m->kv_blocked = false;
    if (chain) {
        if (m->enc_entry.w) {
            CN_TRY(run_chain(m, m->enc_entry, m->x, M, m->qkv, 3 * d, true, CHX_NO_STORE, s, nullptr, 0, blk));
        } else {
            CN_TRY(run_ln(m, m->enc[0].n[0], m->x, m->xn, M, s));
            CN_TRY(run_linear(m, "qkv_proj", m->enc[0].qkv, m->xn, d, m->qkv, 3 * d, 0, M, 0, nullptr, 0, s));
        }
    }
    static const bool no_x3_chain = cn_exp_env("CASSNAT_NO_X3_CHAIN") != nullptr;
    bool x3_rows = !chain && !cap && !no_x3_chain && m->prec == CN_PREC_X3 && !m->enc.empty() && m->enc[0].qkv.px3;
    for (size_t n = 0; x3_rows && n < m->enc.size(); ++n)
        x3_rows = x3_chain_applies(m, m->enc[n], n + 1 < m->enc.size() ? &m->enc[n + 1].qkv : nullptr);
    for (size_t n = 0; n < m->enc.size(); ++n) {
        const Layer& L = m->enc[n];
        const bool last = n + 1 == m->enc.size();
        if (chain) {
            CN_TRY(run_self_attn_core(m, B, Tp, m->keymask, nullptr, 0, s, (n > 0 || m->enc_entry.w) && blk));
            const int xm = cap ? 0 : ((n > 0 ? CHX_IN_BLK : 0) | (last ? CHX_NO_STORE : CHX_OUT_BLK));
            if (last && m->kv_cols > 0) {
                CN_TRY(run_chain(m, m->enc_chain[n], m->x, M, m->kv_all, m->kv_cols, true, xm, s, m->enc_h, d, blk));
                m->kv_ready = true;
                m->kv_blocked = blk;
            } else {
                CN_TRY(run_chain(m, m->enc_chain[n], m->x, M, last ? m->enc_h : m->qkv, last ? d : 3 * d, true, xm, s, nullptr, 0,
                                 blk && !last));
            }
        } else if (x3_rows) {
            if (n == 0) {
                CN_TRY(run_ln(m, L.n[0], m->x, m->xn, M, s));
                CN_TRY(run_linear(m, "qkv_proj", L.qkv, m->xn, d, m->qkv, 3 * d, 0, M, 0, nullptr, 0, s));
            }
            CN_TRY(run_self_attn_core(m, B, Tp, m->keymask, nullptr, 0, s));
            if (last)
                CN_TRY(run_x3_chain(m, L, L.n[1], m->x, M, m->enc_norm, m->enc_h, nullptr, nullptr, 0, "row_chain_x3", s));
            else
                CN_TRY(run_x3_chain(m, L, L.n[1], m->x, M, m->enc[n + 1].n[0], nullptr, &m->enc[n + 1].qkv, m->qkv, 3 * d, "row_chain_x3", s));
        } else {
            CN_TRY(run_self_attn(m, L, n == 0 ? &L.n[0] : nullptr, m->x, B, Tp, m->keymask, nullptr, 0, s));
            CN_TRY(run_ffn(m, L, L.n[1], m->x, M, last ? &m->enc_norm : &m->enc[n + 1].n[0], last ? m->enc_h : m->xn, s));
        }
        if (cap) CN_TRY(capture(m, ("enc_layer" + std::to_string(n)).c_str(), m->x, false, CN_DTYPE_F32, {B, Tp, d}, s));
    }
    if (m->enc.empty()) CN_TRY(run_ln(m, m->enc_norm, m->x, m->enc_h, M, s));
    if (cap) CN_TRY(capture(m, "enc_h", m->enc_h, true, CN_DTYPE_F32, {B, Tp, d}, s));
    return 0;
}

static int stage_decode_tail(cn_model* m, int U, const cn_decode_opts* o, int32_t* hyp, int hyp_stride, int32_t* hyp_len,
                             double* score, hipStream_t s);

static int stage_decode(cn_model* m, int U, const cn_decode_opts* o, int32_t* hyp, int hyp_stride, int32_t* hyp_len,
                        double* score, hipStream_t s) {
    const cn_config& c = m->cfg;
    const int d = c.d_model, B = m->B * m->dec_group, Tp = m->Tp, MU = B * U;
    const bool cap = o->capture != 0;
    m->U = U;
    if (U > m->pe_rows || U < 1 || U > Tp + 1) {
        cn_set_error("decode: token count exceeds the positional table / the frames of the batch");
        return -1;
    }
    CN_TRY(ws_check(m, m->B, m->T, m->dec_group, "decoder side"));
    const bool uni = o->use_unimask != 0;
    static const bool no_chain_p = cn_exp_env("CASSNAT_NO_CHAIN") != nullptr;
    const bool packed = !c.conf_dec && !m->dec_steps.empty() && !no_chain_p && hyp && !cap && !uni && o->beam_width == 1 &&
                        o->reserved[0] == 0 && o->reserved[1] == 0 && !o->no_trigger && m->dec_group == 1;
    m->rows_packed = packed;
    const int* roff = packed ? m->row_off : nullptr;
    const int* rows_dev = packed ? m->row_off + B : nullptr;
    if (packed) {
        CN_TRY(launch_row_plan(m->ylen, B, U, hyp_stride, o->sub_batch, m->ragged ? m->utt_meta : nullptr,
                               m->u_predicted ? m->ymax : nullptr, m->row_off, s));
        CN_TRY(launch_fill_queries_packed(m->pe, m->xd, m->row_off, B, MU, d, s));
    } else {
        CN_TRY(launch_fill_queries(m->pe, m->xd, B, U, d, s));
    }
    auto first_norm_after = [&](int stage, size_t idx) -> const Norm* {
        if (stage == 0 && idx + 1 < m->extra.size()) return &m->extra[idx + 1].n[0];
        if (stage <= 0 && !m->sad.empty()) return &m->sad[0].n[0];
        if (stage == 1 && idx + 1 < m->sad.size()) return &m->sad[idx + 1].n[0];
        if (stage <= 1) return (uni || m->mad.empty()) ? nullptr : &m->mad[0].n[0];
        if (idx + 1 < m->mad.size()) return &m->mad[idx + 1].n[0];
        return nullptr;
    };
    if (c.conf_dec) {
        if (uni) {
            cn_set_error("decode: use_unimask is not defined for the conformer decoder (the reference indexes a tuple there)");
            return -1;
        }
        float* x = m->xd;
        for (size_t i = 0; i < m->extra.size(); ++i) {
            const Layer& L = m->extra[i];
            CN_TRY(launch_convert(m->prec, x, m->xn, (size_t)MU * d, s));
            CN_TRY(run_linear(m, "src_q_proj", L.src_q, m->xn, d, m->qd, d, 0, MU, 0, nullptr, 0, s));
            CN_TRY(run_src_attn_core(m, L, B, U, Tp, m->intervals, s));
            {
                ProfScope ps(m, "out_proj_scaled", 2.0 * MU * d * d, (double)MU * d * (m->es + 4), s);
                GemmArgs g;
                g.A = m->ctx;
                g.lda = d;
                g.W = L.src_o.W;
                g.bias = L.src_o.b;
                g.C = x;
                g.ldc = d;
                g.c_f32 = 1;
                g.M = MU;
// ... 859 lines not shown
```

cassnat_asr_public_amd/csrc/ops.hip:

```cpp
#include <algorithm>
#include <cmath>
#include <cstring>
#include <string>
#include <thread>
#include <vector>

#include "../../include/cassnat_hip.h"
#include "ctc_ngram_search.h"
#include "flac_decode.h"
#include "kernels.h"

namespace {

class Scratch {
  public:
    Scratch(const char* who, hipStream_t s) : who_(who), s_(s) {}
    Scratch(const Scratch&) = delete;
    Scratch& operator=(const Scratch&) = delete;
    ~Scratch() {
        (void)hipStreamSynchronize(s_);
        for (void* p : bufs_) (void)hipFree(p);
    }
    bool ok() const { return ok_; }
    void* alloc(size_t bytes) {
        if (!ok_) return nullptr;
        void* p = nullptr;
        const hipError_t e = hipMalloc(&p, bytes);
        if (e != hipSuccess) return fail("hipMalloc", bytes, e);
        bufs_.push_back(p);
        return p;
    }
    void* upload(const void* host, size_t bytes) {
        void* p = alloc(bytes);
        if (!p) return nullptr;
        const hipError_t e = hipMemcpy(p, host, bytes, hipMemcpyHostToDevice);
        return e == hipSuccess ? p : fail("hipMemcpy", bytes, e);
    }
    int finish(int rc) {
        const hipError_t e = hipStreamSynchronize(s_);
        if (rc == 0 && e != hipSuccess) {
            cn_set_error(std::string(who_) + ": " + hipGetErrorString(e));
            return -2;
        }
        return rc;
    }

  private:
    void* fail(const char* what, size_t bytes, hipError_t e) {
        cn_set_error(std::string(who_) + ": " + what + " of " + std::to_string(bytes) + " bytes failed: " + hipGetErrorString(e));
        ok_ = false;
        return nullptr;
    }
    const char* who_;
    hipStream_t s_;
    std::vector<void*> bufs_;
    bool ok_ = true;
};

std::vector<unsigned char> split_rows256(const float* x, int M) {
    std::vector<unsigned char> hx((size_t)M * 1024);
    for (size_t r = 0; r < (size_t)M; ++r)
        for (size_t c = 0; c < 256; ++c) {
            const float v = x[r * 256 + c];
            const uint16_t hi = cn_host_op16(v);
            const uint32_t hbits = (uint32_t)hi << 16;
            float hf;
            std::memcpy(&hf, &hbits, 4);
            const uint16_t lo = cn_host_op16(v - hf);
            std::memcpy(&hx[r * 1024 + cn_split_off(c)], &hi, 2);
            std::memcpy(&hx[r * 1024 + cn_split_off(c) + 64], &lo, 2);
        }
    return hx;
}

}

static FbankOpts fbank_opts_from(const cn_fbank_opts* o) {
    FbankOpts f;
    f.sample_rate = o->sample_rate;
    f.frame_length_ms = o->frame_length_ms;
    f.frame_shift_ms = o->frame_shift_ms;
    f.preemph = o->preemph;
    f.low_freq = o->low_freq;
    f.high_freq = o->high_freq;
    f.num_mel = o->num_mel;
    f.window_type = o->window_type;
    f.remove_dc = o->remove_dc;
    f.use_power = o->use_power;
    f.use_log = o->use_log;
    return f;
// ... 342 lines not shown
                               int32_t ldv, void* O, int32_t ldo, int32_t B, int32_t H, int32_t Lq, int32_t Lk,
                               const uint8_t* keymask, const int32_t* klen, const int32_t* intervals, int32_t iv_stride,
                               int32_t causal, float scale, void* stream) {
    if ((precision = cn_own_precision(precision, "cn_op_attention")) < 0) return -1;
    AttnArgs a;
    a.Q = Q;
    a.K = K;
    a.V = V;
    a.O = O;
    a.ldq = ldq;
    a.ldk = ldk;
    a.ldv = ldv;
    a.ldo = ldo;
    a.B = B;
    a.H = H;
    a.Lq = Lq;
    a.Lk = Lk;
    a.keymask = keymask;
    a.klen = klen;
    a.intervals = intervals;
    a.iv_stride = iv_stride;
    a.causal = causal;
    a.scale = scale;
    int rc = launch_attention(precision, a, (hipStream_t)stream);
    if (rc == 0 && cn_exp_env("CASSNAT_ATTN_STAMPS")) {
        (void)hipStreamSynchronize((hipStream_t)stream);
        (void)attention_print_stamps();
    }
    return rc;
}

static int op_attention_desc(const char* who, int32_t precision, const cn_attn_desc* d, const int32_t* row_off, int32_t kv_packed,
                             void* stream) {
    if ((precision = cn_own_precision(precision, who)) < 0) return -1;
    if (!d) {
        cn_set_error(std::string(who) + ": null descriptor");
        return -1;
    }
    AttnArgs a;
    a.row_off = row_off;
    a.kv_packed = kv_packed;
    a.Q = d->Q;
    a.K = d->K;
    a.V = d->V;
    a.O = d->O;
    a.ldq = d->ldq;
    a.ldk = d->ldk;
    a.ldv = d->ldv;
    a.ldo = d->ldo;
    a.B = d->B;
    a.H = d->H;
    a.Lq = d->Lq;
    a.Lk = d->Lk;
    a.keymask = d->keymask;
    a.kv_mod = d->kv_mod;
    a.kv_index = d->kv_index;
    a.klen = d->klen;
    a.kcap = d->kcap;
    a.kcap_stride = d->kcap_stride;
    a.q_blocked = d->q_blocked;
    a.kv_blocked = d->kv_blocked;
    a.q_col = d->q_col;
    a.k_col = d->k_col;
    a.v_col = d->v_col;
    a.q_n = d->q_n;
    a.kv_n = d->kv_n;
    a.o_blocked = d->o_blocked;
    a.intervals = d->intervals;
    a.iv_stride = d->iv_stride;
    a.causal = d->causal;
    a.scale = d->scale;
    a.rel_pos = d->rel_pos;
    a.rel_u = d->rel_u;
    a.rel_v = d->rel_v;
    a.rel_R = d->rel_R;
    a.ld_pos = d->ld_pos;
    return launch_attention(precision, a, (hipStream_t)stream);
}

extern "C" int cn_op_attention_desc(int32_t precision, const cn_attn_desc* d, void* stream) {
    return op_attention_desc("cn_op_attention_desc", precision, d, nullptr, 0, stream);
}

extern "C" int cn_op_attention_packed(int32_t precision, const cn_attn_desc* d, const int32_t* row_off_dev, int32_t kv_packed,
                                      void* stream) {
    if (!row_off_dev) {
        cn_set_error("cn_op_attention_packed: null row_off");
        return -1;
    }
    return op_attention_desc("cn_op_attention_packed", precision, d, row_off_dev, kv_packed, stream);
}

extern "C" int cn_op_row_plan(const int32_t* ylen_dev, int32_t B, int32_t U, int32_t hyp_stride, int32_t sub, const int32_t* utt_meta_dev,
                              const int32_t* ymax_dev, int32_t* row_off_dev, void* stream) {
    static_assert(sizeof(UttMeta) == 4 * sizeof(int32_t), "cn_op_row_plan: utt_meta is [B][4] int32");
    if (!ylen_dev || !row_off_dev || B < 1 || U < 0 || sub < 0) {
        cn_set_error("cn_op_row_plan: null argument or B < 1");
        return -1;
    }
    return launch_row_plan(ylen_dev, B, U, hyp_stride, sub, reinterpret_cast<const UttMeta*>(utt_meta_dev), ymax_dev, row_off_dev,
                           (hipStream_t)stream);
}

extern "C" int32_t cn_attn_desc_size(void) { return (int32_t)sizeof(cn_attn_desc); }

extern "C" int cn_op_logsoftmax_argmax(float* logits, int32_t M, int32_t V, int32_t* arg, float* maxlp,
                                       int32_t write_logp, void* stream) {
    return launch_logsoftmax_argmax(logits, M, V, V, arg, maxlp, write_logp, (hipStream_t)stream);
}

extern "C" int cn_op_ctc_align(const int32_t* best, const uint8_t* keymask, const float* size_ratio, int32_t B,
                               int32_t Tp, int32_t blank, int32_t left, int32_t right, int32_t* shift,
                               int32_t* src_size, int32_t* ylen, int32_t* ymax, int32_t* intervals, void* stream) {
    AlignArgs a;
    a.best = best;
    a.keymask = keymask;
    a.size_ratio = size_ratio;
    a.B = B;
    a.Tp = Tp;
    a.blank = blank;
    a.left = left;
    a.right = right;
    a.shift = shift;
    a.src_size = src_size;
    a.ylen = ylen;
    a.ymax = ymax;
    a.intervals = intervals;
    return launch_ctc_align(a, (hipStream_t)stream);
}

extern "C" int cn_op_ctc_prefix_beam(const float* logp, const float* size_ratio, int32_t B, int32_t Tp, int32_t V, int32_t beam,
                                     int32_t pruning, double length_penalty, int32_t blank, int32_t* hyp, int32_t hyp_cap,
                                     int32_t* hyp_len, double* score, double* p_blk, double* p_nblk, int32_t* nbeam, void* stream) {
    hipStream_t s = (hipStream_t)stream;
    const size_t M = (size_t)B * Tp;
    const int P = pruning > 0 ? pruning : 1;
    Scratch sc("cn_op_ctc_prefix_beam", s);
    int* top_idx = (int*)sc.alloc(M * P * 4);
    float* top_val = (float*)sc.alloc(M * P * 4);
    unsigned char* hpar = (unsigned char*)sc.alloc(M * (size_t)std::max(beam, 1));
    int* htok = (int*)sc.alloc(M * (size_t)std::max(beam, 1) * 4);
    if (!sc.ok()) return -2;
    int rc = pruning > 0 ? launch_topk(logp, (int)M, V, V, pruning, top_idx, top_val, s) : 0;
    if (rc == 0) {
        CtcBeamArgs a;
        a.logp = logp;
        a.top_idx = top_idx;
        a.size_ratio = size_ratio;
        a.B = B;
        a.Tp = Tp;
        a.V = V;
        a.P = pruning;
        a.W = beam;
        a.blank = blank;
        a.Lmax = hyp_cap;
        a.lp = length_penalty;
        a.hist_parent = hpar;
        a.hist_tok = htok;
        a.hyp = hyp;
        a.hyp_len = hyp_len;
        a.score = score;
        a.p_blk = p_blk;
        a.p_nblk = p_nblk;
        a.n_out = nbeam;
        rc = launch_ctc_prefix_beam(a, s);
    }
// ... 711 lines not shown
        std::vector<unsigned char> h((size_t)tail_n * 1024);
        pack_proj_x3(wt_host, tail_n, h.data());
        a.tail_p = sc.upload(h.data(), h.size());
        a.tail_b = bt_dev;
        a.tail_out = tail_out_dev;
        a.tail_n = tail_n;
        a.ld_tail = tail_n;
    }
    a.x = x_dev;
    a.ln_a = ln_a_dev;
    a.ln_b = ln_b_dev;
    a.b1 = b1_dev;
    a.b2 = b2_dev;
    a.nln_a = nln_a_dev;
    a.nln_b = nln_b_dev;
    a.xn_out = xn_out_dev;
    a.M = M;
    a.d = 256;
    a.dff = dff;
    a.eps = eps;
    if (!sc.ok()) return -2;
    return sc.finish(launch_ffn_x3(a, (hipStream_t)stream));
}

static int op_chain(float* x_dev, const void* ctx_dev, int32_t ldctx, const float* wo_host, const float* bo_host,
                    const float* ln1_a_host, const float* ln1_b_host, const float* w1_host, const float* b1_host,
                    const float* w2_host, const float* b2_host, const float* nln_a_host, const float* nln_b_host,
                    const float* wt_host, const float* bt_host, void* out_dev, int32_t ldo, int32_t M, int32_t dff,
                    int32_t tail_n, float eps, int32_t x_mode, const int32_t* m_dev, void* stream) {
    if (dff < 0 || dff % 32 != 0 || dff > 2048 || tail_n < 0 || tail_n % 32 != 0 || tail_n > 1536) {
        cn_set_error("cn_op_chain: d_ff and the tail width must be multiples of 32 (<= 2048 / <= 1536)");
        return -1;
    }
    ChainWeights w;
    w.wo = ctx_dev ? wo_host : nullptr;
    w.bo = bo_host;
    w.ln1_a = ln1_a_host;
    w.ln1_b = ln1_b_host;
    w.w1 = w1_host;
    w.b1 = b1_host;
    w.w2 = w2_host;
    w.b2 = b2_host;
    w.nln_a = nln_a_host;
    w.nln_b = nln_b_host;
    w.wt = wt_host;
    w.bt = bt_host;
    w.dff = dff;
    w.tail_n = tail_n;
    const int f8 = (x_mode & 32) != 0;
    if (f8 && (dff <= 0 || dff % 256 != 0 || (x_mode & 8))) {
        cn_set_error("cn_op_chain: the e4m3 feed-forward form (x_mode bit 32) needs d_ff % 256 == 0 and the ReLU activation");
        return -1;
    }
    const size_t units = chain_stream_units(ctx_dev != nullptr, dff, tail_n, f8);
    std::vector<uint16_t> hs((units + 7) * (CHAIN_UNIT_BYTES / 2));
    std::vector<float> ht(CHAIN_TAB_FLOATS + 4);
    int hq[4] = {127, 127, 127, 127};
    pack_chain(w, hs.data(), ht.data(), f8 ? hq : nullptr);
    std::memcpy(&ht[CHAIN_TAB_FLOATS], hq, 16);
    Scratch sc("cn_op_chain", (hipStream_t)stream);
    void* ds = sc.upload(hs.data(), hs.size() * 2);
    const float* dt = (const float*)sc.upload(ht.data(), ht.size() * 4);
    if (!sc.ok()) return -2;
    ChainArgs a;
    a.x = x_dev;
    a.ctx = ctx_dev;
    a.ldctx = ldctx;
    a.wstream = ds;
    a.tab = dt;
    a.out = out_dev;
    a.ldo = ldo;
    a.M = M;
    a.m_dev = m_dev;
    a.d = 256;
    a.dff = dff;
    a.tail_n = tail_n;
    a.has_next = nln_a_host != nullptr;
    a.eps = eps;
    a.x_in_blocked = (x_mode & 1) != 0;
    a.x_out_blocked = (x_mode & 2) != 0;
    a.store_x = (x_mode & 4) == 0;
    a.swish = (x_mode & 8) != 0;
    a.out_blocked = (x_mode & 16) != 0;
    a.f8 = f8;
    a.f8_q = f8 ? reinterpret_cast<const int*>(dt + CHAIN_TAB_FLOATS) : nullptr;
    int rc = launch_chain(a, (hipStream_t)stream);
    if (const char* rep = cn_exp_env("CASSNAT_CHAIN_REPEAT")) {
        const int ns = cn_exp_env("CASSNAT_CHAIN_STREAMS") ? atoi(cn_exp_env("CASSNAT_CHAIN_STREAMS")) : 0;
        std::vector<hipStream_t> ss(ns > 0 ? ns : 0);
        for (auto& q : ss) (void)hipStreamCreateWithFlags(&q, hipStreamNonBlocking);
        (void)hipStreamSynchronize((hipStream_t)stream);
        for (int i = 1; i < atoi(rep) && rc == 0; ++i) rc = launch_chain(a, ns > 0 ? ss[i % ns] : (hipStream_t)stream);
        for (auto& q : ss) {
            (void)hipStreamSynchronize(q);
            (void)hipStreamDestroy(q);
        }
    }
    rc = sc.finish(rc);
    if (cn_exp_env("CASSNAT_CHAIN_STAMPS")) (void)chain_print_stamps();
    return rc;
}

extern "C" int cn_op_chain(float* x_dev, const void* ctx_dev, int32_t ldctx, const float* wo_host, const float* bo_host,
                           const float* ln1_a_host, const float* ln1_b_host, const float* w1_host, const float* b1_host,
                           const float* w2_host, const float* b2_host, const float* nln_a_host, const float* nln_b_host,
                           const float* wt_host, const float* bt_host, void* out_dev, int32_t ldo, int32_t M, int32_t dff,
                           int32_t tail_n, float eps, int32_t x_mode, void* stream) {
    return op_chain(x_dev, ctx_dev, ldctx, wo_host, bo_host, ln1_a_host, ln1_b_host, w1_host, b1_host, w2_host, b2_host, nln_a_host,
                    nln_b_host, wt_host, bt_host, out_dev, ldo, M, dff, tail_n, eps, x_mode, nullptr, stream);
}

extern "C" int cn_op_chain_rows(float* x_dev, const void* ctx_dev, int32_t ldctx, const float* wo_host, const float* bo_host,
                                const float* ln1_a_host, const float* ln1_b_host, const float* w1_host, const float* b1_host,
                                const float* w2_host, const float* b2_host, const float* nln_a_host, const float* nln_b_host,
                                const float* wt_host, const float* bt_host, void* out_dev, int32_t ldo, int32_t M, int32_t dff,
                                int32_t tail_n, float eps, int32_t x_mode, const int32_t* rows_dev, void* stream) {
    if (!rows_dev) {
        cn_set_error("cn_op_chain_rows: null row count");
        return -1;
    }
    return op_chain(x_dev, ctx_dev, ldctx, wo_host, bo_host, ln1_a_host, ln1_b_host, w1_host, b1_host, w2_host, b2_host, nln_a_host,
                    nln_b_host, wt_host, bt_host, out_dev, ldo, M, dff, tail_n, eps, x_mode, rows_dev, stream);
}

static int op_genmax_impl(const void* h_dev, const float* w_host, const float* b_host, int32_t M, int32_t V,
                          int32_t* arg_dev, float* maxlp_dev, const int32_t* tgt_dev, float* tgt_lp_dev, int32_t U, int32_t ld,
                          void* stream) {
    const int vtw = genmax_vtw(V);
    if (vtw > 48) {
        cn_set_error("cn_op_genmax: V too large");
        return -1;
    }
    std::vector<uint16_t> hw((size_t)4 * vtw * 16 * 512);
    std::vector<float> hb((size_t)4 * vtw * 32);
    pack_genmax(w_host, b_host, V, hw.data(), hb.data());
    Scratch sc("cn_op_genmax", (hipStream_t)stream);
    GenmaxArgs a;
    a.h = h_dev;
    a.wp = sc.upload(hw.data(), hw.size() * 2);
    a.bp = (const float*)sc.upload(hb.data(), hb.size() * 4);
    if (!sc.ok()) return -2;
    a.arg = arg_dev;
    a.maxlp = maxlp_dev;
    a.M = M;
    a.V = V;
    a.d = 256;
    a.tgt = tgt_dev;
    a.tgt_lp = tgt_lp_dev;
    a.tgt_U = U;
    a.tgt_ld = ld;
    int rc = launch_genmax(a, (hipStream_t)stream);
    if (const char* rep = cn_exp_env("CASSNAT_GENMAX_REPEAT"))
        for (int i = 1, n = atoi(rep); rc == 0 && i < n; ++i) rc = launch_genmax(a, (hipStream_t)stream);
    return sc.finish(rc);
}

extern "C" int cn_op_genmax(const void* h_dev, const float* w_host, const float* b_host, int32_t M, int32_t V,
                            int32_t* arg_dev, float* maxlp_dev, void* stream) {
    return op_genmax_impl(h_dev, w_host, b_host, M, V, arg_dev, maxlp_dev, nullptr, nullptr, 0, 0, stream);
}

extern "C" int cn_op_genmax_gather(const void* h_dev, const float* w_host, const float* b_host, int32_t B, int32_t U, int32_t V,
                                   const int32_t* tgt_dev, int32_t ld, float* tgt_lp_dev, void* stream) {
    return op_genmax_impl(h_dev, w_host, b_host, B * U, V, nullptr, nullptr, tgt_dev, tgt_lp_dev, U, ld, stream);
}

// ... 60 lines not shown
```

cassnat_asr_public_amd/csrc/sublayers.hip:

```cpp
#include <algorithm>
#include <cmath>

#include "model.h"

namespace cn_host {

int run_linear(cn_model* m, const char* tag, const Linear& l, const void* A, int lda, void* C, int ldc, int c_f32, int M,
               int epi, const float* resid, int ldr, hipStream_t s) {
    ProfScope ps(m, tag, 2.0 * M * l.N * l.K,
                 (double)M * l.K * m->es + (double)l.N * l.K * m->es + (double)M * l.N * (c_f32 ? 4 : m->es), s);
    static const bool no_proj_x3 = cn_exp_env("CASSNAT_NO_PROJ_X3") != nullptr;
    if (l.px3 && m->prec == CN_PREC_X3 && !no_proj_x3 && (epi == 0 || epi == CN_EPI_RESID) && (epi == 0 || c_f32) && lda % 32 == 0 &&
        (c_f32 || ldc % 32 == 0) && (long long)M * std::max(ldc, ldr) * 4 < (1ll << 31)) {
        ProjX3Args a;
        a.A = A;
        a.lda = lda;
        a.wp = l.px3;
        a.bias = l.b;
        a.C = C;
        a.ldc = ldc;
        a.c_f32 = c_f32;
        a.resid = epi == CN_EPI_RESID ? resid : nullptr;
        a.ldr = ldr;
        a.M = M;
// ... 37 lines not shown
        a.act = L.ff_swish ? FF_ACT_SWISH : FF_ACT_RELU;
        a.b1 = L.w1.b;
        a.b2 = L.w2.b;
        if (next) {
            a.nln_a = next->a;
            a.nln_b = next->b;
            a.xn_out = next_out;
        }
        a.M = M;
        a.d = d;
        a.dff = L.w1.N;
        return launch_ffn_x3(a, s);
    }
    if (L.w1p) {
        ProfScope ps(m, "ffn_fused", 4.0 * M * (double)L.w1.N * d,
                     (double)M * d * 8 + 2.0 * L.w1.N * d * 2 + (next ? (double)M * d * 2 : 0.0), s);
        FfnFusedArgs a;
        a.x = x;
        a.ln_a = n.a;
        a.ln_b = n.b;
        a.w1p = L.w1p;
        a.b1 = L.w1.b;
        a.w2p = L.w2p;
        a.b2 = L.w2.b;
        if (next) {
            a.nln_a = next->a;
            a.nln_b = next->b;
            a.xn_out = next_out;
        }
        a.M = M;
        a.d = d;
        a.dff = L.w1.N;
        a.act = L.ff_swish ? FF_ACT_SWISH : FF_ACT_RELU;
        return launch_ffn_fused(a, s);
    }
    CN_TRY(run_ln(m, n, x, m->xn, M, s));
    if (L.ff_swish)
        CN_TRY(run_linear(m, "ffn_w1_swish", L.w1, m->xn, d, m->hbuf, L.w1.N, 0, M, CN_EPI_SWISH, nullptr, 0, s));
    else
        CN_TRY(run_linear(m, "ffn_w1_relu", L.w1, m->xn, d, m->hbuf, L.w1.N, 0, M, CN_EPI_RELU, nullptr, 0, s));
    CN_TRY(run_linear(m, "ffn_w2_resid", L.w2, m->hbuf, L.w1.N, x, d, 1, M, CN_EPI_RESID, x, d, s));
    if (next) CN_TRY(run_ln(m, *next, x, next_out, M, s));
    return 0;
}

bool x3_chain_applies(const cn_model* m, const Layer& L, const Linear* tail) {
    return m->prec == CN_PREC_X3 && L.wx3 && !L.ff_swish && L.self_o.px3 && L.self_o.N == 256 && L.self_o.K == 256 &&
           (!tail || (tail->px3 && tail->K == 256 && tail->N % 128 == 0 && tail->N <= 1024));
}
int run_x3_chain(cn_model* m, const Layer& L, const Norm& n1, float* x, int M, const Norm& next, void* next_out, const Linear* tail,
                 void* tail_out, int ld_tail, const char* tag, hipStream_t s) {
    const int d = m->cfg.d_model, tn = tail ? tail->N : 0;
    const double macs = (double)d * d + 2.0 * d * L.w1.N + (double)d * tn;
    ProfScope ps(m, tag, 2.0 * M * macs, (double)M * d * (4 + 8) + (double)M * (tail ? tn : d) * 4 + 4.0 * macs, s);
    FfnX3Args a;
    a.x = x;
    a.ln_a = n1.a;
    a.ln_b = n1.b;
    a.wst = L.wx3;
    a.mix = ffn_mix_applies();
    a.b1 = L.w1.b;
    a.b2 = L.w2.b;
    a.nln_a = next.a;
    a.nln_b = next.b;
    a.xn_out = next_out;
    a.M = M;
    a.d = d;
    a.dff = L.w1.N;
    a.ctx = m->ctx;
    a.ldctx = d;
    a.wo_p = L.self_o.px3;
    a.bo = L.self_o.b;
    if (tail) {
        a.tail_p = tail->px3;
        a.tail_b = tail->b;
        a.tail_out = tail_out;
        a.tail_n = tn;
        a.ld_tail = ld_tail;
    }
    return launch_ffn_x3(a, s);
}

int run_self_attn_core(cn_model* m, int B, int Lseq, const unsigned char* keymask, const int* klen, int causal,
                       hipStream_t s, bool blocked, const int* row_off) {
    const int d = m->cfg.d_model, M = B * Lseq;
    AttnArgs a;
    const size_t es = m->es;
    a.Q = m->qkv;
    a.K = (const unsigned char*)m->qkv + (size_t)d * es;
    a.V = (const unsigned char*)m->qkv + (size_t)2 * d * es;
    if (blocked) {
        a.K = a.V = m->qkv;
        a.q_blocked = a.kv_blocked = 1;
        a.q_col = 0;
        a.k_col = d;
        a.v_col = 2 * d;
        a.q_n = a.kv_n = 3 * d;
        a.o_blocked = 1;
    }
    m->ctx_blocked = a.o_blocked != 0;
    a.O = m->ctx;
    a.ldq = a.ldk = a.ldv = 3 * d;
    a.ldo = d;
    a.B = B;
    a.H = m->cfg.n_head;
    a.Lq = a.Lk = Lseq;
    a.keymask = keymask;
    a.klen = klen;
    a.row_off = row_off;
    a.kv_packed = row_off ? 1 : 0;
    if (m->ragged && keymask == m->keymask) {
        a.kcap = &m->utt_meta[0].tp;
        a.kcap_stride = (int)(sizeof(UttMeta) / sizeof(int));
    }
    a.causal = causal;
    a.scale = 1.0f / sqrtf((float)(d / m->cfg.n_head));
    ProfScope ps(m, "self_attention", 4.0 * B * a.H * (double)Lseq * Lseq * 64, (double)M * 4 * d * m->es, s);
    return launch_attention(m->prec, a, s);
}

int run_self_attn(cn_model* m, const Layer& L, const Norm* pre, float* x, int B, int Lseq, const unsigned char* keymask,
                  const int* klen, int causal, hipStream_t s) {
    const int d = m->cfg.d_model, M = B * Lseq;
    if (pre) CN_TRY(run_ln(m, *pre, x, m->xn, M, s));
    CN_TRY(run_linear(m, "qkv_proj", L.qkv, m->xn, d, m->qkv, 3 * d, 0, M, 0, nullptr, 0, s));
    CN_TRY(run_self_attn_core(m, B, Lseq, keymask, klen, causal, s));
    CN_TRY(run_linear(m, "out_proj_resid", L.self_o, m->ctx, d, x, d, 1, M, CN_EPI_RESID, x, d, s));
    return 0;
}

int run_chain(cn_model* m, const ChainRef& r, float* x, int M, void* out, int ldo, bool with_next, int x_mode,
              hipStream_t s, void* ln_out, int ld_ln, bool out_blocked, const char* tag, const int* m_dev) {
    const int d = m->cfg.d_model;
    const int tail_n = with_next ? r.tail_n : 0;
    const double macs = (r.has_wo ? (double)d * d : 0.0) + 2.0 * d * r.dff + (double)d * tail_n;
    ProfScope ps(m, tag, 2.0 * M * macs, (double)M * d * (8 + 2) + (double)M * ldo * 2 + 2.0 * macs, s);
    ChainArgs a;
    a.x = x;
    a.ctx = r.has_wo ? m->ctx : nullptr;
    a.ldctx = d;
    a.ctx_blocked = m->ctx_blocked ? 1 : 0;
    a.wstream = r.w;
    a.tab = r.tab;
    a.out = out;
    a.ldo = ldo;
    a.ln_out = ln_out;
    a.ld_ln = ld_ln;
    a.M = M;
    a.m_dev = m_dev;
    a.d = d;
    a.dff = r.dff;
    a.tail_n = tail_n;
    a.has_next = with_next && r.has_next;
    a.x_in_blocked = (x_mode & CHX_IN_BLK) != 0;
    a.x_out_blocked = (x_mode & CHX_OUT_BLK) != 0;
    a.store_x = (x_mode & CHX_NO_STORE) == 0;
    a.swish = r.swish ? 1 : 0;
    a.out_blocked = out_blocked ? 1 : 0;
    a.f8 = r.f8q ? 1 : 0;
    a.f8_q = r.f8q;
    return launch_chain(a, s);
}

constexpr float FP8_S_LN = 16.f, FP8_S_CTX = 16.f, FP8_S_HID = 8.f;
static int run_linear_fp8(cn_model* m, const char* tag, const Linear& l, const void* a8, float a_scale, void* C, int ldc, int c_f32,
                          int c_fp8, float c_scale, int M, int epi, const float* resid, int ldr, hipStream_t s) {
    ProfScope ps(m, tag, 2.0 * M * l.N * l.K, (double)M * l.K + (double)l.N * l.K + (double)M * l.N * (c_f32 ? 4 : (c_fp8 ? 1 : 2)), s);
    GemmArgs g;
    g.A = a8;
    g.lda = l.K;
    g.W = l.W8;
    g.bias = l.b;
    g.C = C;
    g.ldc = ldc;
    g.c_f32 = c_f32;
    g.c_fp8 = c_fp8;
    g.c_scale = c_scale;
    g.M = M;
    g.N = l.N;
    g.K = l.K;
    g.epi = epi;
    g.resid = resid;
    g.ldr = ldr;
    g.ab_fp8 = 1;
    g.acc_scale = 1.f / a_scale;
    g.w_inv_scale = l.w8_inv;
    return launch_gemm(CN_PREC_BF16, g, s);
}

int run_enc_layer_fp8(cn_model* m, const Layer& L, float* x, int B, int Tp, hipStream_t s) {
    const int d = m->cfg.d_model, M = B * Tp;
    void* q8 = m->xn;
    void* h8 = m->hbuf;
    {
        ProfScope ps(m, "layernorm_fp8", 0, (double)M * d * 5, s);
        CN_TRY(launch_layernorm_fp8(x, L.n[0].a, L.n[0].b, q8, M, d, 1e-6f, FP8_S_LN, s));
    }
    CN_TRY(run_linear_fp8(m, "qkv_proj_fp8", L.qkv, q8, FP8_S_LN, m->qkv, 3 * d, 0, 0, 1.f, M, 0, nullptr, 0, s));
    CN_TRY(run_self_attn_core(m, B, Tp, m->keymask, nullptr, 0, s));
    {
        ProfScope ps(m, "quantize_fp8", 0, (double)M * d * 3, s);
        CN_TRY(launch_quantize_fp8(m->ctx, d, q8, M, d, FP8_S_CTX, s));
    }
    CN_TRY(run_linear_fp8(m, "out_proj_fp8", L.self_o, q8, FP8_S_CTX, x, d, 1, 0, 1.f, M, CN_EPI_RESID, x, d, s));
    {
        ProfScope ps(m, "layernorm_fp8", 0, (double)M * d * 5, s);
        CN_TRY(launch_layernorm_fp8(x, L.n[1].a, L.n[1].b, q8, M, d, 1e-6f, FP8_S_LN, s));
    }
    CN_TRY(run_linear_fp8(m, "ffn_w1_fp8", L.w1, q8, FP8_S_LN, h8, L.w1.N, 0, 1, FP8_S_HID, M, CN_EPI_RELU, nullptr, 0, s));
    CN_TRY(run_linear_fp8(m, "ffn_w2_fp8", L.w2, h8, FP8_S_HID, x, d, 1, 0, 1.f, M, CN_EPI_RESID, x, d, s));
    return 0;
}

int run_ffn_swish(cn_model* m, const Linear& w1, const Linear& w2, const Norm& n, float* x, int M, float scale, hipStream_t s) {
    const int d = m->cfg.d_model;
    CN_TRY(run_ln(m, n, x, m->xn, M, s));
    CN_TRY(run_linear(m, "ffn_w1_swish", w1, m->xn, d, m->hbuf, w1.N, 0, M, CN_EPI_SWISH, nullptr, 0, s));
    ProfScope ps(m, "ffn_w2_resid", 2.0 * M * w2.N * w2.K, (double)M * w2.K * m->es + (double)w2.N * w2.K * m->es + (double)M * w2.N * 8, s);
    GemmArgs g;
    g.A = m->hbuf;
    g.lda = w1.N;
    g.W = w2.W;
    g.bias = w2.b;
    g.C = x;
    g.ldc = d;
    g.c_f32 = 1;
    g.M = M;
    g.N = w2.N;
    g.K = w2.K;
    g.epi = CN_EPI_RESID;
    g.resid = x;
    g.ldr = d;
    g.resid_scale = scale;
    return launch_gemm(m->prec, g, s);
}

static int run_rel_attn_core(cn_model* m, const Layer& L, int B, int Lseq, const unsigned char* keymask, const int* klen, hipStream_t s);

int run_rel_self_attn(cn_model* m, const Layer& L, const Norm& n, float* x, int B, int Lseq, const unsigned char* keymask,
                      const int* klen, hipStream_t s) {
    const int d = m->cfg.d_model, M = B * Lseq;
// ... 170 lines not shown
```

cassnat_asr_public_amd/csrc/workspace.hip:

```cpp
#include <algorithm>

#include "model.h"

namespace cn_host {
namespace {

int dev_alloc(cn_model* m, void** p, size_t bytes) {
    if (bytes == 0) bytes = 256;
    CN_HIP_CHECK(hipMalloc(p, bytes));
    m->allocs.push_back(*p);
    return 0;
}

struct WsDims {
    size_t B, Bu, T1, Tp, G;
};
struct WsRow {
    const char* name;
    size_t bytes;
    void (*assign)(cn_model*, void*);
};
#define WS_ROW(field, nbytes)                                                                                             \
    do {                                                                                                                  \
        out.push_back({#field, (nbytes), [](cn_model* h, void* p) { h->field = static_cast<decltype(h->field)>(p); }}); \
    } while (0)
std::vector<WsRow> ws_table(const cn_model* m, const WsDims& v) {
    const cn_config& c = m->cfg;
    const size_t es = m->es;
    const size_t B = v.B, T1 = v.T1, Tp = v.Tp, F1 = m->F1, F2 = m->F2, d = c.d_model, V = c.vocab_size, G = v.G;
    const size_t M0 = B * (Tp + 1);
    const size_t M = M0 * G;
    const size_t dff = std::max(std::max(c.d_encff, c.d_decff), c.d_ff);
    std::vector<WsRow> out;
    WS_ROW(keymask, B * Tp);
    if (c.ast != 2) {
        WS_ROW(c1, B * (T1 + 2) * (F1 + 2) * d * es);
        WS_ROW(c2, B * Tp * F2 * d * es);
    }
    WS_ROW(x, (M + 32) * d * 4);
    WS_ROW(xn, M * d * es);
    WS_ROW(qkv, (M + 32) * 3 * d * es);
    WS_ROW(ctx, (M + 32) * d * es);
    WS_ROW(hbuf, M * dff * es);
    WS_ROW(enc_h, M0 * d * es);
    WS_ROW(kvm, M0 * 2 * d * es);
    if (m->kv_cols > 0) WS_ROW(kv_all, (M0 + 32) * (size_t)m->kv_cols * es);
    WS_ROW(qd, (M + 32) * d * es);
    WS_ROW(dec_h, M * d * es);
    WS_ROW(xd, (M + 32) * d * 4);
    WS_ROW(xd2, (M + 32) * d * 4);
    WS_ROW(logits, M0 * V * 4);
    WS_ROW(best, M * 4);
    WS_ROW(ctc_maxlp, M0 * 4);
    WS_ROW(shift, M * 4);
    WS_ROW(src_size, v.Bu * G * 4);
    WS_ROW(ylen, v.Bu * G * 4);
    WS_ROW(utt_meta, v.Bu * sizeof(UttMeta));
    WS_ROW(row_off, (v.Bu * G + 1) * 4);
    WS_ROW(ymax, 256);
    WS_ROW(intervals, B * G * (Tp + 1) * 16);
    WS_ROW(tok, M * 4);
    WS_ROW(val, M * 4);
    WS_ROW(topk_idx, M0 * 16 * 4);
    WS_ROW(topk_val, M0 * 16 * 4);
    if (c.conf_enc || c.conf_dec) {
        WS_ROW(cv_a, M * 2 * d * es);
        WS_ROW(cv_f, M * d * 4);
        WS_ROW(gn_stats, v.Bu * G * 2 * 8);
    }
    return out;
}
#undef WS_ROW

}

int build_workspace(cn_model* m) {
    if (m->keymask) return 0;
    const WsDims dims = {(size_t)m->maxB, (size_t)m->maxU, (size_t)m->maxT1, (size_t)m->maxTp, (size_t)std::max(1, m->cfg.esa_group)};
    for (const WsRow& row : ws_table(m, dims)) {
        void* p = nullptr;
        CN_TRY(dev_alloc(m, &p, row.bytes));
        row.assign(m, p);
        m->ws_cap[row.name] = row.bytes;
    }
    CN_HIP_CHECK(hipHostMalloc((void**)&m->ymax_pinned, 64, hipHostMallocDefault));
    CN_HIP_CHECK(hipHostMalloc((void**)&m->ymax_ring, 64, hipHostMallocDefault));
    bool range_guard = false;
#ifdef CN_OP16_F16
    range_guard = true;
#else
    range_guard = conv2_mix_applies(m->prec, m->cfg.d_model, m->cfg.d_model) && m->cfg.ast != 2;
#endif
    if (range_guard) {
        CN_HIP_CHECK(hipHostMalloc((void**)&m->op16_fault, 64, hipHostMallocMapped));
        *m->op16_fault = 0;
    }
    return 0;
}

int ws_check(cn_model* m, int B, int T, int G, const char* what) {
    const int T1 = (T - 1) / 2 + 1, Tp = (T1 - 1) / 2 + 1;
    for (const WsRow& row : ws_table(m, {(size_t)B, (size_t)B, (size_t)T1, (size_t)Tp, (size_t)std::max(1, G)})) {
        auto it = m->ws_cap.find(row.name);
        if (it == m->ws_cap.end() || row.bytes > it->second) {
            cn_set_error(std::string(what) + ": workspace buffer '" + row.name + "' holds " +
                         std::to_string(it == m->ws_cap.end() ? 0 : it->second) + " bytes, the call (B=" + std::to_string(B) + " T=" +
                         std::to_string(T) + " alignments=" + std::to_string(G) + ") needs " + std::to_string(row.bytes) +
                         " (workspace: max_batch " + std::to_string(m->maxB) + " x max_frames " + std::to_string(m->maxT) + ")");
            return -1;
        }
    }
    if (Tp + 1 > m->pe_rows) {
        cn_set_error(std::string(what) + ": more subsampled frames than the positional table has rows");
        return -1;
    }
    return 0;
}

int capture(cn_model* m, const char* name, const void* src, bool model_prec, int dtype, std::vector<int64_t> shape,
            hipStream_t s) {
    size_t n = 1;
    for (auto v : shape) n *= (size_t)v;
    const size_t esz = dtype == CN_DTYPE_U8 ? 1 : (dtype == CN_DTYPE_F64 ? 8 : 4);
// ... 31 lines not shown
```

cassnat_asr_public_amd/hip.py:

```python
import ctypes as C
import os

import numpy as np

from . import abi

_HERE = os.path.dirname(os.path.abspath(__file__))
LIB_PATH = os.environ.get("CASSNAT_HIP_LIB") or os.path.join(_HERE, "libcassnat_hip.so")
LIB_PATH_F16 = os.path.join(_HERE, "libcassnat_hip_f16.so")
HEADER_PATH = abi.HEADER_PATH

_K = abi.CONSTANTS
_F32, _BF16, _FP8, _BF16X3, _F16 = (_K["CN_PRECISION_" + n] for n in ("F32", "BF16", "FP8", "BF16X3", "F16"))
PRECISION = {"fp32": _F32, "f32": _F32, "float32": _F32, "bf16": _BF16, "bfloat16": _BF16, "fp8": _FP8, "bf16x3": _BF16X3, "fp16": _F16,
             "float16": _F16}
DTYPES = {_K["CN_DTYPE_F32"]: np.float32, _K["CN_DTYPE_I32"]: np.int32, _K["CN_DTYPE_U8"]: np.uint8, _K["CN_DTYPE_F64"]: np.float64}
FP8_SCOPE_BITS = {"conv2": _K["CN_FP8_CONV2"], "linear": _K["CN_FP8_LINEAR"], "ffn": _K["CN_FP8_FFN"]}


def parse_fp8_scope(text):
    text = (text or "all").strip().lower()
    if text == "all":
        return 0, 0
    scope, first = 0, 0
# ... 211 lines not shown

def flac_scratch_bytes(frames, frame_words):
    return int(lib().cn_flac_scratch_bytes(int(frames), int(frame_words)))


def flac_decode(staged, staged_bytes, table, frames, utt, utts, max_channels, frame_words, pcm, pcm_bytes, status, scratch=None):
    assert staged.is_contiguous() and staged.element_size() == 1 and 0 <= int(staged_bytes) <= staged.numel()
    assert table.is_contiguous() and table.element_size() == 4 and table.numel() >= 4 * int(frames)
    assert utt.is_contiguous() and utt.element_size() == 4 and utt.numel() >= 3 * int(utts)
    assert pcm.is_contiguous() and 0 <= int(pcm_bytes) <= pcm.numel() * pcm.element_size() and status.element_size() == 4
    check(lib().cn_op_flac_decode(_ptr(staged), int(staged_bytes), _ptr(table), int(frames), _ptr(utt), int(utts), int(max_channels),
                                  int(frame_words), _ptr(pcm), int(pcm_bytes), _ptr(status), _ptr(scratch),
                                  0 if scratch is None else scratch.numel() * scratch.element_size(), current_stream()), "cn_op_flac_decode")
    return pcm


class Engine:

    def __init__(self, args, precision="bf16", max_batch=32, max_frames=2048, device=0, esa_group=1, share_with=None):
        self.L = lib_for(precision)
        ast = int(getattr(args, "ast", 0))
        self.cfg = CnConfig(
            input_size=args.input_size, d_model=args.d_model, n_head=args.n_head, d_encff=args.d_encff,
            d_decff=args.d_decff, n_enc=args.N_enc, n_extra=args.N_extra, n_self_dec=args.N_self_dec,
            n_mix_dec=args.N_mix_dec, vocab_size=args.vocab_size, precision=PRECISION[precision],
            max_batch=max_batch, max_frames=max_frames, device=device, ast=ast,
            conf_enc=int(getattr(args, "conf_enc", 0)), conf_dec=int(getattr(args, "conf_dec", 0)),
            enc_max_rel=int(getattr(args, "enc_max_rel", 0)), dec_max_rel=int(getattr(args, "dec_max_rel", 0)),
            enc_kernel=int(getattr(args, "enc_kernel", 0)), dec_kernel=int(getattr(args, "dec_kernel", 0)),
            d_ff=int(getattr(args, "d_ff", 0)), esa_group=int(esa_group),
            fp8_scope=int(getattr(args, "fp8_scope", 0)), fp8_ffn_first_layer=int(getattr(args, "fp8_ffn_first_layer", 0)))
        self.precision = precision
        self.handle = C.c_void_p()
        if share_with is not None:
            if not share_with.finalized or not share_with.handle:
                raise HipError("share_with needs a finalized engine")
            self._chk(self.L.cn_model_create_shared(C.byref(self.cfg), share_with.handle, C.byref(self.handle)), "cn_model_create_shared")
            self.finalized = True
        else:
            self._chk(self.L.cn_model_create(C.byref(self.cfg), C.byref(self.handle)), "cn_model_create")
            self.finalized = False

    def _chk(self, rc, what=""):
        check(rc, what, self.L)

    def close(self):
        if getattr(self, "handle", None):
            self.L.cn_model_destroy(self.handle)
            self.handle = None

    def __del__(self):
        try:
            self.close()
        except Exception:
            pass

    def load_state(self, state, pe_table):
        for name, w in state.items():
            a = np.ascontiguousarray(w.detach().cpu().numpy() if hasattr(w, "detach") else w, dtype=np.float32)
            shape = (C.c_int64 * a.ndim)(*a.shape)
            self._chk(self.L.cn_model_load_weights(self.handle, name.encode(), a.ctypes.data_as(C.c_void_p), shape, a.ndim),
                  f"load {name}")
        pe = np.ascontiguousarray(pe_table.detach().cpu().numpy() if hasattr(pe_table, "detach") else pe_table,
                                  dtype=np.float32)
        self._chk(self.L.cn_model_load_pe(self.handle, pe.ctypes.data_as(C.c_void_p), pe.shape[0]), "load pe")
        self.finalize()

    def finalize(self):
        self._chk(self.L.cn_model_finalize(self.handle), "cn_model_finalize")
        self.finalized = True

    def weight_blob(self):
        p, n = C.c_void_p(), C.c_int64()
        self._chk(self.L.cn_model_weight_blob(self.handle, C.byref(p), C.byref(n)), "cn_model_weight_blob")
        return p.value, n.value

    @staticmethod
    def make_opts(args, capture=False):
        opts = CnDecodeOpts(padding_idx=int(args.padding_idx), sos=1, left_trigger=int(getattr(args, "left_trigger", 0)),
                            right_trigger=int(getattr(args, "right_trigger", 0)), src_trigger=int(bool(getattr(args, "src_trigger", False))),
                            use_unimask=int(bool(getattr(args, "use_unimask", False))), beam_width=int(args.beam_width),
                            capture=int(bool(capture)), no_trigger=int(not getattr(args, "use_trigger", True)))
        opts.reserved[1] = int(bool(getattr(args, "hip_padded_rows", False)))
        return opts

    def decode(self, feats, size_ratio, opts, hyp, hyp_len, score):
        B, T, F = feats.shape
        self._chk(self.L.cn_decode_nast(self.handle, _ptr(feats), _ptr(size_ratio), B, T, F, C.byref(opts), _ptr(hyp),
                                    hyp.shape[1], _ptr(hyp_len), _ptr(score), current_stream()), "cn_decode_nast")

    def decode_merged(self, feats, size_ratio, opts, sub_rows, sub_frames, hyp, hyp_len, score, u_hint=0):
        B, T, F = feats.shape
        n = len(sub_rows) if sub_rows is not None else 0
        rows = (C.c_int32 * max(1, n))(*[int(x) for x in (sub_rows or [])])
        frames = (C.c_int32 * max(1, n))(*[int(x) for x in (sub_frames or [])])
        ticket = C.c_int32(-1)
        self._chk(self.L.cn_decode_nast_merged(self.handle, _ptr(feats), _ptr(size_ratio), B, T, F, C.byref(opts), n, rows, frames,
                                           int(u_hint), _ptr(hyp), hyp.shape[1], _ptr(hyp_len), _ptr(score), current_stream(),
                                           C.byref(ticket)), "cn_decode_nast_merged")
        return ticket.value

    def check_range(self, what="decode"):
        if self.precision not in ("fp16", "float16", "bf16x3"):
            return
        fault, limit = C.c_int32(), C.c_float()
        self._chk(self.L.cn_take_range_fault(self.handle, C.byref(fault), C.byref(limit)), "cn_take_range_fault")
        if fault.value and self.precision == "bf16x3":
            raise HipError(f"{what}: features beyond the range the split-bf16 engine's mixed-arithmetic convolution holds at its "
                           f"tolerance (|x| > {limit.value:.4g} lets conv1 outputs pass the e4m3 operands' 448): normalise the features "
                           "(CMVN) or decode with --hip_precision fp32")
        if fault.value:
            raise HipError(f"{what}: features beyond the fp16 engine's half-precision range (|x| > {limit.value:.4g} lets a subsampling "
                           "convolution's output pass 65504 / 2): normalise the features (CMVN) or decode with --hip_precision bf16 / bf16x3")

    def ticket(self, t):
        ymax, used = C.c_int32(), C.c_int32()
        self._chk(self.L.cn_decode_ticket(self.handle, int(t), C.byref(ymax), C.byref(used)), "cn_decode_ticket")
        return ymax.value, used.value

    def encode_align(self, feats, size_ratio, opts):
        B, T, F = feats.shape
        ymax = C.c_int32()
        self._chk(self.L.cn_encode_align(self.handle, _ptr(feats), _ptr(size_ratio), B, T, F, C.byref(opts),
                                     C.byref(ymax), current_stream()), "cn_encode_align")
        return ymax.value

    def ast_begin(self, feats, opts, want_ctc, max_len, max_slots, ctc_beam):
        B, T, F = feats.shape
        self._chk(self.L.cn_ast_begin(self.handle, _ptr(feats), B, T, F, C.byref(opts), int(want_ctc), max_len, max_slots,
                                  ctc_beam, current_stream()), "cn_ast_begin")

    def ast_step(self, pos, tok, utt, anc, keyok, temperature, K, topk_idx, topk_val):
        self._chk(self.L.cn_ast_step(self.handle, tok.shape[0], pos, _ptr(tok), _ptr(utt), _ptr(anc), _ptr(keyok), anc.shape[1],
                                 float(temperature), K, _ptr(topk_idx), _ptr(topk_val), current_stream()), "cn_ast_step")

    def ast_attach_lm(self, lm):
        if lm is not None and lm.L is not self.L:
            raise HipError("cn_ast_attach_lm: the LM engine comes from the other library")
        self._chk(self.L.cn_ast_attach_lm(self.handle, lm.handle if lm is not None else None), "cn_ast_attach_lm")
        self._lm = lm

    def ast_step_lm(self, pos, tok, utt, anc, keyok, temperature, K, lm_weight, use_ctc, topk_idx, topk_val, lm_val=None):
        self._chk(self.L.cn_ast_step_lm(self.handle, tok.shape[0], pos, _ptr(tok), _ptr(utt), _ptr(anc), _ptr(keyok), anc.shape[1],
                                    float(temperature), K, float(lm_weight), int(use_ctc), _ptr(topk_idx), _ptr(topk_val),
                                    _ptr(lm_val) if lm_val is not None else None, current_stream()), "cn_ast_step_lm")

    def nat_attach_lm(self, lm):
        if lm is not None and lm.L is not self.L:
            raise HipError("cn_nat_attach_lm: the LM engine comes from the other library")
        self._chk(self.L.cn_nat_attach_lm(self.handle, lm.handle if lm is not None else None), "cn_nat_attach_lm")
        self._lm = lm

    def nat_lm_finish(self, opts, ymax, beam_width, lm_weight, length_penalty, zero_past_len, hyp, hyp_len, score):
        self._chk(self.L.cn_nat_lm_finish(self.handle, C.byref(opts), int(ymax), int(beam_width), float(lm_weight),
                                          int(length_penalty is not None), float(length_penalty or 0.0), int(bool(zero_past_len)),
                                          _ptr(hyp), hyp.shape[2], _ptr(hyp_len), _ptr(score), current_stream()), "cn_nat_lm_finish")

    def lm_step_begin(self, max_len, max_slots):
        self._chk(self.L.cn_lm_step_begin(self.handle, int(max_len), int(max_slots)), "cn_lm_step_begin")

    def lm_step(self, pos, tok, anc, keyok, logp):
        self._chk(self.L.cn_lm_step(self.handle, tok.shape[0], pos, _ptr(tok), _ptr(anc), _ptr(keyok), anc.shape[1], _ptr(logp),
                                current_stream()), "cn_lm_step")

    def ast_ctc_score(self, out_len, utt, last_tok, cand, prev_ref, parity, eos, score):
        self._chk(self.L.cn_ast_ctc_score(self.handle, cand.shape[0], out_len, _ptr(utt), _ptr(last_tok), _ptr(cand), cand.shape[1],
# ... 128 lines not shown
```

Before: 52330 utt/s.

## Fuse encoder QKV projection into the resident self-attention kernel

Adds a projecting form of the resident 8-wave attention kernel. Each (utterance, head) block loads the layer-normed rows and that head's Q/K/V weight tiles, computes the projections with MFMA, and writes K/V into LDS and Q into registers. The encoder chain kernel now emits only a blocked LayerNorm output instead of computing and storing the full QKV tensor, removing that write and re-read. The cost is that the LN input is read once per head, and the attention kernel does more compute and needs more barriers per block. It applies only to bf16 with 4 heads and 128 < Tp <= 256, and it also adds a standalone op entry point.

Measured after the change: 53540 utt/s (median of 6 runs). +2.3%, better.

```diff
diff --git a/cassnat_asr_public_amd/abi.py b/cassnat_asr_public_amd/abi.py
--- a/cassnat_asr_public_amd/abi.py
+++ b/cassnat_asr_public_amd/abi.py
@@ -99,10 +99,13 @@
 EXTRA_HEADER_PATH = os.path.join(os.path.dirname(HEADER_PATH), "cassnat_hip_ctc_ngram.h")
 with open(EXTRA_HEADER_PATH) as _f:
     EXTRA_FUNCTIONS = parse(_f.read(), base=HEADER).functions
+PROJ_HEADER_PATH = os.path.join(os.path.dirname(HEADER_PATH), "cassnat_hip_attention_proj.h")
+with open(PROJ_HEADER_PATH) as _f:
+    PROJ_FUNCTIONS = parse(_f.read(), base=HEADER).functions
 
 
 def bind(L):
-    for name, (restype, argtypes) in list(FUNCTIONS.items()) + list(EXTRA_FUNCTIONS.items()):
+    for name, (restype, argtypes) in list(FUNCTIONS.items()) + list(EXTRA_FUNCTIONS.items()) + list(PROJ_FUNCTIONS.items()):
         fn = getattr(L, name)
         fn.restype, fn.argtypes = restype, argtypes
     return L
diff --git a/cassnat_asr_public_amd/build.py b/cassnat_asr_public_amd/build.py
--- a/cassnat_asr_public_amd/build.py
+++ b/cassnat_asr_public_amd/build.py
@@ -25,7 +25,7 @@
 
 def build(force=False, verbose=False, extra_flags=(), lib=LIB, objdir=None):
     headers = [os.path.join(CSRC, h) for h in os.listdir(CSRC) if h.endswith(".h")]
-    headers += [os.path.join(os.path.dirname(CSRC), "..", "include", h) for h in ("cassnat_hip.h", "cassnat_hip_ctc_ngram.h")]
+    headers += [os.path.join(os.path.dirname(CSRC), "..", "include", h) for h in ("cassnat_hip.h", "cassnat_hip_ctc_ngram.h", "cassnat_hip_attention_proj.h")]
     objdir = objdir or os.path.join(CSRC, "build")
     os.makedirs(objdir, exist_ok=True)
 
diff --git a/cassnat_asr_public_amd/csrc/attention.hip b/cassnat_asr_public_amd/csrc/attention.hip
--- a/cassnat_asr_public_amd/csrc/attention.hip
+++ b/cassnat_asr_public_amd/csrc/attention.hip
@@ -33,6 +33,9 @@
     int rel_R, ld_pos;
     const int* row_off;
     int kv_packed;
+    const unsigned char* Y;
+    const unsigned char* W;
+    const float* bt;
 };
 
 template <typename T> struct AttnCfg;
@@ -59,12 +62,13 @@
 __device__ long long attn_stamps[8];
 #define AT_STAMP(i) if (p.stamps && blockIdx.x == 0 && blockIdx.y == gridDim.y - 1 && blockIdx.z == gridDim.z - 1 && threadIdx.x == 0) attn_stamps[i] = (long long)__builtin_amdgcn_s_memtime();
 
-template <typename T, int NW, bool RES, bool REL = false, bool PK = false>
+template <typename T, int NW, bool RES, bool REL = false, bool PK = false, bool PROJ = false>
 __global__ __launch_bounds__(64 * NW, (RES && NW == 8) ? 4 : ((__is_same(T, split_t) && NW == 4 && !REL) ? 2 : 1)) void attention_kernel(AttnParams p) {
     typedef AttnCfg<T> Cfg;
     typedef typename Frag<T>::type frag_t;
     constexpr bool SPLIT = __is_same(T, split_t);
     static_assert(!SPLIT || !RES, "split-bf16 attention: the staged forms only");
+    static_assert(!PROJ || (RES && NW == 8 && !REL && !PK && sizeof(T) == 2), "the projecting form: resident, 8 waves, 16-bit operands");
     constexpr int KROW = Cfg::KROW, CPR = Cfg::CPR;
     constexpr int VROW = RES ? 128 : Cfg::VROW;
     constexpr int KT_BYTES = 64 * KROW, VT_BYTES = (SPLIT ? 2 : 1) * 64 * VROW, NRES = RES ? 4 : 1;
@@ -79,7 +83,14 @@
 
     const int tid = threadIdx.x, lane = tid & 63, wave = tid >> 6;
     const int half = lane >> 5, l31 = lane & 31;
-    const int b = blockIdx.z, h = blockIdx.y;
+    int b = blockIdx.z, h = blockIdx.y;
+    if constexpr (PROJ) {
+        const int id = blockIdx.y + 4 * blockIdx.z, grp = id >> 5, r = id & 31;
+        if (grp < ((int)gridDim.z >> 3)) {
+            b = grp * 8 + (r & 7);
+            h = r >> 3;
+        }
+    }
     AT_STAMP(0)
     const long long q0 = PK ? (long long)p.row_off[b] : (long long)b * p.Lq;
     const int Lq = PK ? p.row_off[b + 1] - p.row_off[b] : p.Lq;
@@ -93,7 +104,9 @@
     frag_t qf[NF];
     {
         const unsigned char* qp = p.Q + (q0 + qc) * p.ldq_b + (long long)h * KROW;
-        if constexpr (SPLIT) {
+        if constexpr (PROJ) {
+            (void)qp;
+        } else if constexpr (SPLIT) {
 #pragma unroll
             for (int s = 0; s < NF; ++s) {
                 const unsigned char* c = qp + (s >> 1) * 128 + (2 * (s & 1) + half) * 16;
@@ -116,6 +129,85 @@
 #pragma unroll
             for (int s = 0; s < NF; ++s) qf[s] = as_frag<T>(ld16(qp + (2 * s + half) * 16));
         }
+    }
+    if constexpr (PROJ) {
+        typedef unsigned u32x4 __attribute__((ext_vector_type(4)));
+        const long long ym = q0 + qc;
+        int y_half = half;
+        asm volatile("" : "+v"(y_half));
+        const int y_lane = ((y_half << 5) + (int)(ym & 31)) * 16;
+        const unsigned char* yb = p.Y + (ym >> 5) * 16384 + y_lane;
+        const int key = wave * 32 + l31;
+        bf16x8 yf[16];
+#pragma unroll
+        for (int ks = 0; ks < 16; ++ks) yf[ks] = as_frag<bf16>(ld16(yb + ks * 1024));
+        uint4 wr[4];
+        auto fetch = [&](int tile) {
+            const uint4* src = reinterpret_cast<const uint4*>(p.W) + (long long)tile * 1024 + tid;
+#pragma unroll
+            for (int i = 0; i < 4; ++i) wr[i] = src[NT * i];
+        };
+        auto put = [&]() {
+#pragma unroll
+            for (int i = 0; i < 4; ++i) st16(Ks_all + (tid + NT * i) * 16, wr[i]);
+        };
+        auto project = [&](int tile, int d, u32x4& o_0, u32x4& o_1) {
+            f32x16 a;
+#pragma unroll
+            for (int g = 0; g < 4; ++g) {
+                const f32x4 v = *reinterpret_cast<const f32x4*>(p.bt + 32 * tile + 8 * g + 4 * half);
+#pragma unroll
+                for (int e = 0; e < 4; ++e) a[4 * g + e] = v[e];
+            }
+#pragma unroll
+            for (int ks = 0; ks < 16; ++ks)
+                a = CN_MFMA16(as_frag<bf16>(ld16(Ks_all + d * 16384 + ks * 1024 + lane * 16)), yf[ks], a, 0, 0, 0);
+#pragma unroll
+            for (int gp = 0; gp < 2; ++gp) {
+                bf16x4 o0, o1;
+#pragma unroll
+                for (int e = 0; e < 4; ++e) {
+                    o0[e] = (bf16)a[8 * gp + e];
+                    o1[e] = (bf16)a[8 * gp + 4 + e];
+                }
+                const uint2 lo_ = __builtin_bit_cast(uint2, o0), hi_ = __builtin_bit_cast(uint2, o1);
+                const auto s0_ = __builtin_amdgcn_permlane32_swap(lo_.x, hi_.x, false, false);
+                const auto s1_ = __builtin_amdgcn_permlane32_swap(lo_.y, hi_.y, false, false);
+                (gp ? o_1 : o_0) = u32x4{s0_[0], s1_[0], s0_[1], s1_[1]};
+            }
+        };
+        u32x4 pk[4];
+        fetch(16 + 2 * h);
+        put();
+        __syncthreads();
+#pragma unroll
+        for (int d = 0; d < 2; ++d) {
+            project(16 + 2 * h + d, d, pk[0], pk[1]);
+#pragma unroll
+            for (int c = 0; c < 2; ++c)
+                *reinterpret_cast<u32x4*>(Vs_all + key * 128 + (((2 * (2 * d + c) + half) ^ (((key >> 1) & 1) << 2)) << 4)) = pk[c];
+        }
+        __syncthreads();
+        fetch(2 * h);
+        put();
+        __syncthreads();
+#pragma unroll
+        for (int d = 0; d < 2; ++d) {
+            project(2 * h + d, d, pk[0], pk[1]);
+            qf[2 * d] = __builtin_bit_cast(bf16x8, pk[0]);
+            qf[2 * d + 1] = __builtin_bit_cast(bf16x8, pk[1]);
+        }
+        __syncthreads();
+        fetch(8 + 2 * h);
+        put();
+        __syncthreads();
+        project(8 + 2 * h, 0, pk[0], pk[1]);
+        project(8 + 2 * h + 1, 1, pk[2], pk[3]);
+        __syncthreads();
+#pragma unroll
+        for (int c = 0; c < 4; ++c)
+            *reinterpret_cast<u32x4*>(Ks_all + key * KROW + (((2 * c + half) ^ Cfg::swz(key)) << 4)) = pk[c];
+        AT_STAMP(1)
     }
     constexpr int REL_N = REL ? 64 : 1;
     __shared__ float rel_tab[REL ? 64 * 64 : 1];
@@ -239,7 +331,7 @@
     if constexpr (RES) {
         const int wave_u = __builtin_amdgcn_readfirstlane(wave);
         const int r8 = lane >> 3, cp = lane & 7;
-        for (int piece = wave_u; piece < nkt * 16; piece += NW) {
+        for (int piece = wave_u; !PROJ && piece < nkt * 16; piece += NW) {
             const int kt2 = piece >> 4, is_v = (piece >> 3) & 1, j = piece & 7;
             const int row = 8 * j + r8;
             int key = kt2 * 64 + row;
@@ -254,7 +346,7 @@
             __builtin_amdgcn_global_load_lds((const __attribute__((address_space(1))) void*)src,
                                              (__attribute__((address_space(3))) void*)dst, 16, 0, 0);
         }
-        AT_STAMP(1)
+        if constexpr (!PROJ) AT_STAMP(1)
         if (tid < NRES) Mplain[tid] = 1;
         __syncthreads();
         for (int i = tid; i < nkt * 64; i += NT) {
@@ -568,6 +660,9 @@
     }
     p.row_off = a.row_off;
     p.kv_packed = a.kv_packed;
+    p.Y = (const unsigned char*)a.proj_y;
+    p.W = (const unsigned char*)a.proj_w;
+    p.bt = a.proj_b;
     if ((a.row_off && (a.rel_pos || sizeof(T) != 2 || __is_same(T, split_t))) ||
         (a.kv_packed && (!a.row_off || a.kv_mod > 0 || a.kv_index || a.keymask || a.Lq != a.Lk))) {
         cn_set_error("attention: packed rows exist for the 16-bit kernels without relative positions; packed keys are the entry's own "
@@ -592,6 +687,21 @@
             hipLaunchKernelGGL((attention_kernel<T, 2, false, true>), dim3(cn_ceil_div(a.Lq, 64), a.H, a.B), dim3(128), 0, s, p);
             CN_HIP_CHECK(hipGetLastError());
             return 0;
+        }
+    }
+    if (a.proj_y) {
+        if constexpr (sizeof(T) == 2) {
+            if (!a.proj_w || !a.proj_b || a.H != 4 || a.Lq != a.Lk || a.Lk > 256 || a.row_off || a.rel_pos || a.kv_mod > 0 || a.kv_index) {
+                cn_set_error("attention: the projecting form is self attention of at most 256 rows per entry, 4 heads (d_model 256), "
+                             "without packed rows, relative positions, kv_mod or kv_index");
+                return -1;
+            }
+            hipLaunchKernelGGL((attention_kernel<T, 8, true, false, false, true>), dim3(1, a.H, a.B), dim3(512), 0, s, p);
+            CN_HIP_CHECK(hipGetLastError());
+            return 0;
+        } else {
+            cn_set_error("attention: the projecting form exists for the 16-bit kernels");
+            return -1;
         }
     }
     const long long big_grid = (long long)cn_ceil_div(a.Lq, 128) * a.H * a.B;
@@ -644,7 +754,8 @@
         }
     }
     const long long w = 64LL * a.H;
-    if ((!a.q_blocked && a.ldq < w) || (!a.kv_blocked && (a.ldk < w || a.ldv < w)) || a.ldo < w) {
+    const bool qkv_used = a.proj_y == nullptr;
+    if ((qkv_used && ((!a.q_blocked && a.ldq < w) || (!a.kv_blocked && (a.ldk < w || a.ldv < w)))) || a.ldo < w) {
         cn_set_error("attention: row strides ldq / ldk / ldv / ldo must be >= 64 * H");
         return -1;
     }
diff --git a/cassnat_asr_public_amd/csrc/chain.hip b/cassnat_asr_public_amd/csrc/chain.hip
--- a/cassnat_asr_public_amd/csrc/chain.hip
+++ b/cassnat_asr_public_amd/csrc/chain.hip
@@ -17,6 +17,7 @@
 constexpr int CT_BO = 0, CT_LN1A = 256, CT_LN1B = 512, CT_B2 = 768, CT_NLNA = 1024, CT_NLNB = 1280, CT_BT = 1536,
               CT_B1 = 3072;
 constexpr int CH_MAX_TAIL = 48, CH_MAX_FFN_TILES = 64;
+static_assert(CT_BT == CHAIN_TAB_BT && CH_TAB_FLOATS == CHAIN_TAB_FLOATS && CH_UNIT_BYTES == CHAIN_UNIT_BYTES, "kernels.h names the same layout");
 
 __device__ long long ch_stamps[16];
 
@@ -43,6 +44,7 @@
     int ctx_blk;
     const int* f8_q;
     const int* m_dev;
+    int ln_blk;
 };
 
 #define CH_STR2(x) #x
@@ -830,6 +832,13 @@
         ch_layernorm_pack<false>(acc, tab_lane, CT_NLNA, CT_NLNB, 0, p.eps, bop);
         CH_STAMP(7)
         if (p.ln_out) {
+            if (p.ln_blk) {
+                if (rb < nrb) {
+                    bf16x8* op = reinterpret_cast<bf16x8*>(p.ln_out) + ((long long)rb * 16 * 64 + lane);
+#pragma unroll
+                    for (int k = 0; k < 16; ++k) op[k * 64] = bop[k];
+                }
+            } else
             if (live) {
                 bf16* op = p.ln_out + (long long)m * p.ld_ln + 4 * half;
 #pragma unroll
@@ -998,6 +1007,11 @@
     p.out_blk = a.out_blocked && a.tail_n > 0;
     p.ctx_blk = a.ctx && a.ctx_blocked;
     p.f8_q = a.f8_q;
+    p.ln_blk = a.ln_blocked && p.ln_out && a.has_next;
+    if (p.ln_blk && p.ld_ln != CH_D) {
+        cn_set_error("chain: a blocked LNn(x) has 256 columns");
+        return -1;
+    }
     if (p.ctx_blk && a.ldctx != CH_D) {
         cn_set_error("chain: a blocked ctx has 256 columns");
         return -1;
diff --git a/cassnat_asr_public_amd/csrc/kernels.h b/cassnat_asr_public_amd/csrc/kernels.h
--- a/cassnat_asr_public_amd/csrc/kernels.h
+++ b/cassnat_asr_public_amd/csrc/kernels.h
@@ -112,6 +112,9 @@
     const float* rel_pos = nullptr;
     const float *rel_u = nullptr, *rel_v = nullptr;
     int rel_R = 0, ld_pos = 0;
+    const void* proj_y = nullptr;
+    const void* proj_w = nullptr;
+    const float* proj_b = nullptr;
 };
 int launch_attention(int prec, const AttnArgs& a, hipStream_t s);
 int attention_print_stamps();
@@ -275,6 +278,7 @@
                      hipStream_t s);
 
 constexpr int CHAIN_TAB_FLOATS = 5120;
+constexpr int CHAIN_TAB_BT = 1536;
 constexpr int CHAIN_UNIT_BYTES = 16384;
 struct ChainArgs {
     float* x = nullptr;
@@ -291,6 +295,7 @@
     const int* m_dev = nullptr;
     int x_in_blocked = 0, x_out_blocked = 0, store_x = 1;
     int out_blocked = 0;
+    int ln_blocked = 0;
     int swish = 0;
     int f8 = 0;
     const int* f8_q = nullptr;
diff --git a/cassnat_asr_public_amd/csrc/model.h b/cassnat_asr_public_amd/csrc/model.h
--- a/cassnat_asr_public_amd/csrc/model.h
+++ b/cassnat_asr_public_amd/csrc/model.h
@@ -239,13 +239,13 @@
 int run_x3_chain(cn_model* m, const Layer& L, const Norm& n1, float* x, int M, const Norm& next, void* next_out, const Linear* tail,
                  void* tail_out, int ld_tail, const char* tag, hipStream_t s);
 int run_self_attn_core(cn_model* m, int B, int Lseq, const unsigned char* keymask, const int* klen, int causal, hipStream_t s,
-                       bool blocked = false, const int* row_off = nullptr);
+                       bool blocked = false, const int* row_off = nullptr, const ChainRef* proj = nullptr);
 int run_self_attn(cn_model* m, const Layer& L, const Norm* pre, float* x, int B, int Lseq, const unsigned char* keymask,
                   const int* klen, int causal, hipStream_t s);
 enum { CHX_IN_BLK = 1, CHX_OUT_BLK = 2, CHX_NO_STORE = 4 };
 int run_chain(cn_model* m, const ChainRef& r, float* x, int M, void* out, int ldo, bool with_next, int x_mode, hipStream_t s,
               void* ln_out = nullptr, int ld_ln = 0, bool out_blocked = false, const char* tag = "row_chain",
-              const int* m_dev = nullptr);
+              const int* m_dev = nullptr, bool ln_only = false);
 int run_enc_layer_fp8(cn_model* m, const Layer& L, float* x, int B, int Tp, hipStream_t s);
 int run_ffn_swish(cn_model* m, const Linear& w1, const Linear& w2, const Norm& n, float* x, int M, float scale, hipStream_t s);
 int run_rel_self_attn(cn_model* m, const Layer& L, const Norm& n, float* x, int B, int Lseq, const unsigned char* keymask,
diff --git a/cassnat_asr_public_amd/csrc/model.hip b/cassnat_asr_public_amd/csrc/model.hip
--- a/cassnat_asr_public_amd/csrc/model.hip
+++ b/cassnat_asr_public_amd/csrc/model.hip
@@ -192,8 +192,14 @@
     const bool chain = !m->enc.empty() && m->enc_chain.size() == m->enc.size() && !no_chain;
     static const bool blk = cn_exp_env("CASSNAT_NO_BLOCKED_QKV") == nullptr;
     m->kv_blocked = false;
+    static const bool no_attn_proj = cn_exp_env("CASSNAT_NO_ATTN_PROJ") != nullptr;
+    bool proj = chain && !cap && blk && !no_attn_proj && o->reserved[2] == 0 && m->enc_entry.w && m->prec == CN_PREC_BF16 &&
+                c.n_head == 4 && Tp > 128 && Tp <= 256 && m->enc_entry.tail_n == 3 * d;
+    for (size_t n = 0; proj && n + 1 < m->enc_chain.size(); ++n) proj = m->enc_chain[n].tail_n == 3 * d && m->enc_chain[n].has_next;
     if (chain) {
-        if (m->enc_entry.w) {
+        if (m->enc_entry.w && proj) {
+            CN_TRY(run_chain(m, m->enc_entry, m->x, M, m->xn, d, true, CHX_NO_STORE, s, nullptr, 0, false, "row_chain", nullptr, true));
+        } else if (m->enc_entry.w) {
             CN_TRY(run_chain(m, m->enc_entry, m->x, M, m->qkv, 3 * d, true, CHX_NO_STORE, s, nullptr, 0, blk));
         } else {
             CN_TRY(run_ln(m, m->enc[0].n[0], m->x, m->xn, M, s));
@@ -208,12 +214,17 @@
         const Layer& L = m->enc[n];
         const bool last = n + 1 == m->enc.size();
         if (chain) {
-            CN_TRY(run_self_attn_core(m, B, Tp, m->keymask, nullptr, 0, s, (n > 0 || m->enc_entry.w) && blk));
+            if (proj)
+                CN_TRY(run_self_attn_core(m, B, Tp, m->keymask, nullptr, 0, s, false, nullptr, n > 0 ? &m->enc_chain[n - 1] : &m->enc_entry));
+            else
+                CN_TRY(run_self_attn_core(m, B, Tp, m->keymask, nullptr, 0, s, (n > 0 || m->enc_entry.w) && blk));
             const int xm = cap ? 0 : ((n > 0 ? CHX_IN_BLK : 0) | (last ? CHX_NO_STORE : CHX_OUT_BLK));
             if (last && m->kv_cols > 0) {
                 CN_TRY(run_chain(m, m->enc_chain[n], m->x, M, m->kv_all, m->kv_cols, true, xm, s, m->enc_h, d, blk));
                 m->kv_ready = true;
                 m->kv_blocked = blk;
+            } else if (proj && !last) {
+                CN_TRY(run_chain(m, m->enc_chain[n], m->x, M, m->xn, d, true, xm, s, nullptr, 0, false, "row_chain", nullptr, true));
             } else {
                 CN_TRY(run_chain(m, m->enc_chain[n], m->x, M, last ? m->enc_h : m->qkv, last ? d : 3 * d, true, xm, s, nullptr, 0,
                                  blk && !last));
diff --git a/cassnat_asr_public_amd/csrc/ops.hip b/cassnat_asr_public_amd/csrc/ops.hip
--- a/cassnat_asr_public_amd/csrc/ops.hip
+++ b/cassnat_asr_public_amd/csrc/ops.hip
@@ -6,6 +6,7 @@
 #include <vector>
 
 #include "../../include/cassnat_hip.h"
+#include "../../include/cassnat_hip_attention_proj.h"
 #include "ctc_ngram_search.h"
 #include "flac_decode.h"
 #include "kernels.h"
@@ -514,6 +515,53 @@
     return op_attention_desc("cn_op_attention_desc", precision, d, nullptr, 0, stream);
 }
 
+extern "C" int cn_op_attention_proj(int32_t precision, const cn_attn_desc* d, const void* y_dev, const float* wt_host,
+                                    const float* bt_host, void* stream) {
+    if ((precision = cn_own_precision(precision, "cn_op_attention_proj")) < 0) return -1;
+    if (!d || !y_dev || !wt_host || !bt_host) {
+        cn_set_error("cn_op_attention_proj: null argument");
+        return -1;
+    }
+    if (precision != CN_PREC_BF16) {
+        cn_set_error("cn_op_attention_proj: the projecting form exists for the 16-bit kernels");
+        return -1;
+    }
+    ChainWeights w;
+    w.wt = wt_host;
+    w.bt = bt_host;
+    w.tail_n = 768;
+    std::vector<uint16_t> hs(chain_stream_units(0, 0, 768) * (CHAIN_UNIT_BYTES / 2));
+    std::vector<float> ht(CHAIN_TAB_FLOATS);
+    pack_chain(w, hs.data(), ht.data());
+    Scratch sc("cn_op_attention_proj", (hipStream_t)stream);
+    const void* ds = sc.upload(hs.data(), hs.size() * 2);
+    const float* dt = (const float*)sc.upload(ht.data(), ht.size() * 4);
+    if (!sc.ok()) return -2;
+    AttnArgs a;
+    a.O = d->O;
+    a.ldo = d->ldo;
+    a.B = d->B;
+    a.H = d->H;
+    a.Lq = d->Lq;
+    a.Lk = d->Lk;
+    a.keymask = d->keymask;
+    a.kv_mod = d->kv_mod;
+    a.kv_index = d->kv_index;
+    a.klen = d->klen;
+    a.kcap = d->kcap;
+    a.kcap_stride = d->kcap_stride;
+    a.o_blocked = d->o_blocked;
+    a.intervals = d->intervals;
+    a.iv_stride = d->iv_stride;
+    a.causal = d->causal;
+    a.scale = d->scale;
+    a.rel_pos = d->rel_pos;
+    a.proj_y = y_dev;
+    a.proj_w = ds;
+    a.proj_b = dt + CHAIN_TAB_BT;
+    return sc.finish(launch_attention(precision, a, (hipStream_t)stream));
+}
+
 extern "C" int cn_op_attention_packed(int32_t precision, const cn_attn_desc* d, const int32_t* row_off_dev, int32_t kv_packed,
                                       void* stream) {
     if (!row_off_dev) {
@@ -1391,6 +1439,7 @@
     a.store_x = (x_mode & 4) == 0;
     a.swish = (x_mode & 8) != 0;
     a.out_blocked = (x_mode & 16) != 0;
+    a.ln_blocked = (x_mode & 64) != 0;
     a.f8 = f8;
     a.f8_q = f8 ? reinterpret_cast<const int*>(dt + CHAIN_TAB_FLOATS) : nullptr;
     int rc = launch_chain(a, (hipStream_t)stream);
diff --git a/cassnat_asr_public_amd/csrc/sublayers.hip b/cassnat_asr_public_amd/csrc/sublayers.hip
--- a/cassnat_asr_public_amd/csrc/sublayers.hip
+++ b/cassnat_asr_public_amd/csrc/sublayers.hip
@@ -143,7 +143,7 @@
 }
 
 int run_self_attn_core(cn_model* m, int B, int Lseq, const unsigned char* keymask, const int* klen, int causal,
-                       hipStream_t s, bool blocked, const int* row_off) {
+                       hipStream_t s, bool blocked, const int* row_off, const ChainRef* proj) {
     const int d = m->cfg.d_model, M = B * Lseq;
     AttnArgs a;
     const size_t es = m->es;
@@ -157,6 +157,13 @@
         a.k_col = d;
         a.v_col = 2 * d;
         a.q_n = a.kv_n = 3 * d;
+        a.o_blocked = 1;
+    }
+    if (proj) {
+        a.proj_y = m->xn;
+        a.proj_w = (const unsigned char*)proj->w +
+                   chain_stream_units(proj->has_wo, proj->dff, 0, proj->f8q != nullptr) * (size_t)CHAIN_UNIT_BYTES;
+        a.proj_b = proj->tab + CHAIN_TAB_BT;
         a.o_blocked = 1;
     }
     m->ctx_blocked = a.o_blocked != 0;
@@ -176,7 +183,8 @@
     }
     a.causal = causal;
     a.scale = 1.0f / sqrtf((float)(d / m->cfg.n_head));
-    ProfScope ps(m, "self_attention", 4.0 * B * a.H * (double)Lseq * Lseq * 64, (double)M * 4 * d * m->es, s);
+    ProfScope ps(m, "self_attention", 4.0 * B * a.H * (double)Lseq * Lseq * 64 + (proj ? 2.0 * M * d * 3.0 * d : 0.0),
+                 proj ? (double)M * 2 * d * m->es + (double)B * 3 * d * d * m->es : (double)M * 4 * d * m->es, s);
     return launch_attention(m->prec, a, s);
 }
 
@@ -191,9 +199,9 @@
 }
 
 int run_chain(cn_model* m, const ChainRef& r, float* x, int M, void* out, int ldo, bool with_next, int x_mode,
-              hipStream_t s, void* ln_out, int ld_ln, bool out_blocked, const char* tag, const int* m_dev) {
+              hipStream_t s, void* ln_out, int ld_ln, bool out_blocked, const char* tag, const int* m_dev, bool ln_only) {
     const int d = m->cfg.d_model;
-    const int tail_n = with_next ? r.tail_n : 0;
+    const int tail_n = with_next && !ln_only ? r.tail_n : 0;
     const double macs = (r.has_wo ? (double)d * d : 0.0) + 2.0 * d * r.dff + (double)d * tail_n;
     ProfScope ps(m, tag, 2.0 * M * macs, (double)M * d * (8 + 2) + (double)M * ldo * 2 + 2.0 * macs, s);
     ChainArgs a;
@@ -218,6 +226,7 @@
     a.store_x = (x_mode & CHX_NO_STORE) == 0;
     a.swish = r.swish ? 1 : 0;
     a.out_blocked = out_blocked ? 1 : 0;
+    a.ln_blocked = ln_only ? 1 : 0;
     a.f8 = r.f8q ? 1 : 0;
     a.f8_q = r.f8q;
     return launch_chain(a, s);
diff --git a/cassnat_asr_public_amd/csrc/workspace.hip b/cassnat_asr_public_amd/csrc/workspace.hip
--- a/cassnat_asr_public_amd/csrc/workspace.hip
+++ b/cassnat_asr_public_amd/csrc/workspace.hip
@@ -38,7 +38,7 @@
         WS_ROW(c2, B * Tp * F2 * d * es);
     }
     WS_ROW(x, (M + 32) * d * 4);
-    WS_ROW(xn, M * d * es);
+    WS_ROW(xn, (M + 32) * d * es);
     WS_ROW(qkv, (M + 32) * 3 * d * es);
     WS_ROW(ctx, (M + 32) * d * es);
     WS_ROW(hbuf, M * dff * es);
diff --git a/cassnat_asr_public_amd/hip.py b/cassnat_asr_public_amd/hip.py
--- a/cassnat_asr_public_amd/hip.py
+++ b/cassnat_asr_public_amd/hip.py
@@ -317,6 +317,7 @@
                             use_unimask=int(bool(getattr(args, "use_unimask", False))), beam_width=int(args.beam_width),
                             capture=int(bool(capture)), no_trigger=int(not getattr(args, "use_trigger", True)))
         opts.reserved[1] = int(bool(getattr(args, "hip_padded_rows", False)))
+        opts.reserved[2] = int(bool(getattr(args, "hip_chain_qkv", False)))
         return opts
 
     def decode(self, feats, size_ratio, opts, hyp, hyp_len, score):
diff --git a/include/cassnat_hip_attention_proj.h b/include/cassnat_hip_attention_proj.h
--- /dev/null
+++ b/include/cassnat_hip_attention_proj.h
@@ -0,0 +1,14 @@
+#ifndef CASSNAT_HIP_ATTENTION_PROJ_H
+#define CASSNAT_HIP_ATTENTION_PROJ_H
+#include "cassnat_hip.h"
+#ifdef __cplusplus
+extern "C" {
+#endif
+
+int cn_op_attention_proj(int32_t precision, const cn_attn_desc* a, const void* y_dev, const float* wt_host, const float* bt_host,
+                         void* stream);
+
+#ifdef __cplusplus
+}
+#endif
+#endif
```
